# huangnengCSU/longcallR

Measured on AMD Instinct MI355X. Metric: candidate_sites_per_sec, higher is better.
Workload: dtype u8 in, u32 counts, f64 likelihoods, i64 fixed-point phase scores

## Files before the change

longcallr_amd/api.py:

```python
import ctypes as C

import numpy as np

from . import _abi, _lib
from ._lib import LcrError


def _view(ptr, dtype, n):
    if n == 0 or not ptr:
        return np.zeros(0, dtype=dtype)
    buf = (C.c_char * (np.dtype(dtype).itemsize * n)).from_address(ptr)
    return np.frombuffer(buf, dtype=dtype, count=n).copy()


def _view_nocopy(ptr, dtype, n):
    if n == 0 or not ptr:
        return np.zeros(0, dtype=dtype)
    buf = (C.c_char * (np.dtype(dtype).itemsize * n)).from_address(ptr)
    return np.frombuffer(buf, dtype=dtype, count=n)


_DEBUG_ENV = {"LCR_PHASE_PROF": "phase_prof", "LCR_GRID_MIN_ENTRIES": "grid_min_entries",
              "LCR_GRID_GENERIC": "grid_generic", "LCR_GRID_SPEC_LANES": "grid_spec_lanes", "LCR_GRID_SPEC_BATCH": "grid_spec_batch", "LCR_POST_HALF": "post_half", "LCR_ENUM_FORCE_BIG": "enum_force_big",
              "LCR_ENUM_FORCE_STREAM": "enum_force_stream", "LCR_ENUM_ELIDE": "enum_elide", "LCR_HIST_TILES": "hist_tiles", "LCR_TIE_ARITH": "tie_arith", "LCR_CHAIN_TIES": "chain_ties", "LCR_K3_HITS": "k3_hits", "LCR_FUSE_FILTER": "fuse_filter", "LCR_ASYNC_PHASE": "async_phase", "LCR_HOST_TRACE": "host_trace", "LCR_OWN_FILL": "own_fill", "LCR_REDO_LDS": "redo_lds", "LCR_SPEC_COMPACT": "spec_compact", "LCR_LEAN_PLANES": "lean_planes"}


class Engine:
    def __init__(self, device=0, params=None, timing=False):
        self.lib = _lib.load()
        h = C.c_void_p()
        rc = self.lib.lcr_ctx_create(device, C.byref(h))
        if rc != 0:
            raise LcrError("lcr_ctx_create(device=%d) failed with %d: no usable HIP device; "
                           "liblcr has no CPU fallback" % (device, rc))
        self.h = h
        self.device = device
        self.params = params if params is not None else _abi.make_params()
        self._sites = None
        self._keep = None
        self.last_truncated_columns = 0
        if timing:
            self.lib.lcr_enable_timing(self.h, 1)
            if timing is not True:
                self.debug_set("timing_mask", sum(1 << int(k) for k in timing))
        import os
        for env, key in _DEBUG_ENV.items():
            v = os.environ.get(env)
            if v is not None:
                self.debug_set(key, int(v) if v.lstrip("-").isdigit() else 1)
        if os.environ.get("LCR_LOCK_DIR"):
            self._chk(self.lib.lcr_ctx_set_lock_dir(self.h, os.fsencode(os.environ["LCR_LOCK_DIR"])), "lcr_ctx_set_lock_dir")

    def debug_set(self, key, value):
        self._chk(self.lib.lcr_debug_set(self.h, key.encode(), int(value)), "lcr_debug_set")
        return self

    def close(self):
        if getattr(self, "h", None):
            self.lib.lcr_ctx_destroy(self.h)
            self.h = None

    __del__ = close

    def _chk(self, rc, what):
        if rc != 0:
            raise LcrError("%s failed (%d): %s" % (what, rc, self.lib.lcr_last_error(self.h).decode()))

    def set_stream(self, hip_stream_ptr):
        self._chk(self.lib.lcr_ctx_set_stream(self.h, C.c_void_p(hip_stream_ptr)), "lcr_ctx_set_stream")

    def sync(self):
        self._chk(self.lib.lcr_ctx_sync(self.h), "lcr_ctx_sync")
        self._sites = None

    def set_async_phase(self, on=True):
        rc = self.lib.lcr_ctx_set_async_phase(self.h, 1 if on else 0)
        self.async_warning = self.lib.lcr_last_error(self.h).decode() if rc > 0 else None
        if rc < 0:
            self._chk(rc, "lcr_ctx_set_async_phase")
        return self

    def load_batch(self, batch):
        if isinstance(batch, _abi.ReadBatch):
            reads, regions = batch.c_reads(), batch.c_regions()
            self._keep = (batch, reads, regions)
        else:
            reads, regions, keep = batch
            self._keep = (keep, reads, regions)
        self._chk(self.lib.lcr_load_batch(self.h, C.byref(reads), C.byref(regions)), "lcr_load_batch")
        return self

    def load_batch_async(self, batch, slot):
        reads, regions = batch.c_reads(), batch.c_regions()
        if not hasattr(self, "_keep_slot"):
            self._keep_slot = {}
        self._chk(self.lib.lcr_load_batch_async(self.h, C.byref(reads), C.byref(regions), int(slot)), "lcr_load_batch_async")
        self._keep_slot[int(slot)] = (batch, reads, regions)
        return self

    def bind_batch(self, slot):
        self._chk(self.lib.lcr_bind_batch(self.h, int(slot)), "lcr_bind_batch")
        return self

    def discover_regions(self, ref_start, ref_end, contig_len, truncation=False, truncation_coverage=200000):
        if not 0 <= int(truncation_coverage) < 1 << 32:
            raise ValueError("truncation_coverage must be in [0, 2^32), got %r" % (truncation_coverage,))
        rs = np.ascontiguousarray(ref_start, dtype=np.int32)
        re_ = np.ascontiguousarray(ref_end, dtype=np.int32)
        o = _abi.LcrRegionList()
        nt = C.c_int64(0)
        self._chk(self.lib.lcr_discover_regions_truncated(self.h, _abi.LCR_MEM_HOST, int(rs.size), rs.ctypes.data, re_.ctypes.data,
                                                          int(contig_len), 1 if truncation else 0, int(truncation_coverage), C.byref(o),
                                                          C.byref(nt)), "lcr_discover_regions_truncated")
        self.last_truncated_columns = int(nt.value)
        return list(zip(_view(o.start0, np.int64, o.n_regions).tolist(), _view(o.len, np.int32, o.n_regions).tolist(),
                        _view(o.max_cov, np.uint32, o.n_regions).tolist()))

    def fill_data_into_freq_vec(self):
        self._chk(self.lib.lcr_pileup(self.h, C.byref(self.params)), "lcr_pileup")
        return self

    def get_candidate_snps(self):
        self._chk(self.lib.lcr_candidates(self.h, C.byref(self.params)), "lcr_candidates")
        return self

    def import_external_candidates(self, pos0, genotype, qual):
        if any(getattr(t, "is_cuda", False) for t in (pos0, genotype, qual)):
            import torch
            ts = (pos0, genotype, qual)
            want = (torch.int64, torch.uint8, torch.float32)
            if not all(getattr(t, "is_cuda", False) for t in ts):
                raise ValueError("device sites: pos0, genotype and qual must all be device tensors")
            for name, t, dt in zip(("pos0", "genotype", "qual"), ts, want):
                if t.dtype != dt:
                    raise ValueError("device sites: %s must be %s, got %s" % (name, dt, t.dtype))
                if t.device.index != self.device:
                    raise ValueError("device sites: %s is on %s, the engine on device %d" % (name, t.device, self.device))
                if t.dim() != 1 or not t.is_contiguous():
                    raise ValueError("device sites: %s must be a contiguous 1-d tensor" % name)
            if len({t.numel() for t in ts}) != 1:
                raise ValueError("pos0, genotype and qual must have the same length")
            self._release_sites()
            torch.cuda.current_stream(self.device).synchronize()
            self._chk(self.lib.lcr_import_candidates(self.h, C.byref(self.params), _abi.LCR_MEM_DEVICE, int(pos0.numel()),
                                                     *[C.c_void_p(t.data_ptr()) for t in ts]), "lcr_import_candidates")
            self._sites = ts
            return self
        p = np.ascontiguousarray(pos0, dtype=np.int64)
        g = np.ascontiguousarray(genotype, dtype=np.uint8)
        q = np.ascontiguousarray(qual, dtype=np.float32)
        if not (p.size == g.size == q.size):
            raise ValueError("pos0, genotype and qual must have the same length")
        self._release_sites()
        self._chk(self.lib.lcr_import_candidates(self.h, C.byref(self.params), _abi.LCR_MEM_HOST, int(p.size), p.ctypes.data, g.ctypes.data,
                                                 q.ctypes.data), "lcr_import_candidates")
        return self

    def _release_sites(self):
        if self._sites is not None:
            self.sync()

    def get_fragments(self):
        self._chk(self.lib.lcr_fragments(self.h, C.byref(self.params)), "lcr_fragments")
        self._sites = None
        return self

    def phase(self):
        self._chk(self.lib.lcr_phase(self.h, C.byref(self.params)), "lcr_phase")
        return self

    def junctions(self, min_count=10, min_junctions=2):
        p = _abi.LcrJunctionParams(int(min_count), int(min_junctions))
        self._chk(self.lib.lcr_junctions(self.h, C.byref(p)), "lcr_junctions")
        o = _abi.LcrJunctionList()
        self._chk(self.lib.lcr_get_junctions(self.h, C.byref(o)), "lcr_get_junctions")
        return _view(o.junc, _abi.JUNC_DTYPE, o.n_junctions), _view(o.junc_region_off, np.int32, o.n_regions + 1)

# ... 194 lines not shown
```

longcallr_amd/csrc/k4_enum.hip:

```cpp
#include <climits>
#include <type_traits>
#include "k4_dev.h"
#include "k4_grid.h"
#include "k4_kernels.h"

#ifndef ENUM_OCC
#define ENUM_OCC 3
#endif
namespace {

struct EnumTile { int32_t slot; uint32_t e0, ne; };
__device__ __forceinline__ EnumTile enum_tile_of(const PhaseDev& P, const EnumSpan* __restrict__ spans, int n_spans, uint32_t per, bool winner) {
  EnumTile t;
  const uint32_t bid = blockIdx.x;
  if (winner) { t.slot = spans[bid].slot; t.e0 = 0; t.ne = 1; return t; }
  const int lane = threadIdx.x & 63;
  int lo = 0, hi = n_spans;
  if (n_spans <= 4096) {
    const int step = (n_spans + 63) / 64;
    const int i1 = lane * step;
    const unsigned long long m1 = __ballot(i1 < n_spans && spans[min(i1, n_spans - 1)].tile0 <= bid);
    const int seg = __popcll(m1) - 1;
    lo = seg * step; hi = min(n_spans, lo + step);
    const int i2 = lo + lane;
    const unsigned long long m2 = __ballot(i2 < hi && spans[min(i2, n_spans - 1)].tile0 <= bid);
    lo = lo + __popcll(m2) - 1;
  } else {
    while (hi - lo > 1) { const int mid = (lo + hi) >> 1; if (spans[mid].tile0 <= bid) lo = mid; else hi = mid; }
  }
  t.slot = spans[lo].slot;
  const uint32_t n = 1u << P.reg[t.slot].S;
  t.e0 = (bid - spans[lo].tile0) * per;
  t.ne = min(per, n - t.e0);
  return t;
}

#if defined(ENUM_PROF) && ENUM_PROF == 2
#define ENUM_PROF_STEPS 1
#define ENUM_STEP(k) do { prof_steps[k] += (unsigned long long)E; } while (0)
#define ENUM_STEP_FLUSH(base) do { if (lane == 0) for (int k = 0; k < 4; k++) atomicAdd(&P.tie_ctr[(base) + k], prof_steps[k]); } while (0)
#else
#define ENUM_STEP(k) do { } while (0)
#define ENUM_STEP_FLUSH(base) do { } while (0)
#endif
#if defined(ENUM_PROF) && !defined(ENUM_PROF_STEPS)
#define ENUM_PROF_TIMES 1
#define ENUM_PT(i) do { if (threadIdx.x == 0) atomicMax(&P.tie_ctr[i], (unsigned long long)((long long)wall_clock64() - prof_t0)); } while (0)
#else
#define ENUM_PT(i) do { } while (0)
#endif
__global__ void __launch_bounds__(64 * ENUM_WAVES)
k4_enum_resolve(PhaseDev P, const EnumSpan* __restrict__ spans, const int64_t* __restrict__ job_base, const long long* __restrict__ job_obj,
                const int64_t* __restrict__ st_base, const unsigned long long* __restrict__ st_words) {
  extern __shared__ __attribute__((aligned(16))) uint8_t lds[];
  const long long prof_t0 = (long long)wall_clock64(); (void)prof_t0;
  const int slot = spans[blockIdx.x].slot;
  const RegionDev rd = P.reg[slot];
  const int tid = threadIdx.x, nt = blockDim.x, lane = tid & 63, wave = tid >> 6;
  const int R = rd.R, S = rd.S;
  const uint32_t E = (uint32_t)P.prow_ptr[rd.rp_off + R];
  const uint32_t n_jobs = 1u << S;
  const long long* const o = job_obj + job_base[slot];
  const unsigned long long* const st = st_words + st_base[slot];
  const uint32_t nk = (uint32_t)(R + 63) / 64, sw = enum_state_words((uint32_t)R);
  const ResolveLayout L = resolve_layout((uint32_t)R, E, (uint32_t)S);
  uint16_t* rp = (uint16_t*)(lds + L.rp);
  uint16_t* ent16 = (uint16_t*)(lds + L.ent16);
  double* lut = (double*)(lds + L.lut);
  double* pse = (double*)(lds + L.pse);
  unsigned long long* sg_ref = (unsigned long long*)(lds + L.sg_ref);
  unsigned long long* hetw = (unsigned long long*)(lds + L.hetw);
  unsigned long long* repmask = (unsigned long long*)(lds + L.repmask);
  uint32_t* rowsnps = (uint32_t*)(lds + L.rowsnps);
  __shared__ uint32_t s_adj[32], s_grp[32];
  uint32_t* t_e = (uint32_t*)(lds + L.res);
  double* t_sum = (double*)(lds + L.res + 8 * ENUM_TCAP);
  constexpr uint32_t EVCAP = 96;
  double* ev_t = (double*)(lds + L.res + 16 * ENUM_TCAP);
  uint16_t* ev_x = (uint16_t*)(lds + L.res + 16 * ENUM_TCAP + 8 * EVCAP);
  __shared__ uint32_t s_nev;
  __shared__ long long s_best[ENUM_WAVES];
  __shared__ uint32_t s_wcnt[ENUM_WAVES], s_dif[ENUM_WAVES], s_ntied;
  const uint32_t TLCAP = resolve_tlcap((uint32_t)S);
  uint16_t* tl = (uint16_t*)(lds + L.res + 16 * ENUM_TCAP + 96 * 10 + 16);
  __shared__ uint32_t s_win, s_wj[ENUM_WAVES], s_first;
  __shared__ double s_winsum, s_wsum[ENUM_WAVES];
  __shared__ int s_flat;
  auto ld_obj = [&](uint32_t e) { return o[e]; };
  auto ld_st = [&](uint32_t e, uint32_t w) { return st[(size_t)e * sw + w]; };
  if (tid < 64) lut[tid] = (tid & 31) < 31 ? (tid < 32 ? P.lut64->le[tid] : P.lut64->l1e[tid - 32]) : 0.0;
  { const int32_t* g_rp = P.prow_ptr + rd.rp_off; for (int r = tid; r <= R; r += nt) rp[r] = (uint16_t)g_rp[r]; }
  for (int e = tid; e < (int)E; e += nt) {
    const uint32_t v = P.pval[rd.e_off + e];
    ent16[e] = (uint16_t)(((uint32_t)P.pcol[rd.e_off + e] & 31u) | (v & 32u) | ((v & 31u) << 6));
  }
  __syncthreads();
  for (int r = tid; r < R; r += nt) if (rp[r + 1] > rp[r]) ent16[rp[r + 1] - 1] |= 0x800u;
  ENUM_PT(0);
  constexpr int OV = 4;
  long long ov[OV];
  long long best = LLONG_MIN;
#pragma unroll
  for (int k = 0; k < OV; k++) { const uint32_t e = (uint32_t)tid + (uint32_t)k * 256u; ov[k] = e < n_jobs ? ld_obj(e) : LLONG_MIN; }
#pragma unroll
  for (int k = 0; k < OV; k++) if (ov[k] > best) best = ov[k];
  for (uint32_t e = tid + OV * 256u; e < n_jobs; e += nt) { const long long v = ld_obj(e); if (v > best) best = v; }
  for (int d = 32; d >= 1; d >>= 1) { const long long ob = __shfl_xor(best, d, 64); if (ob > best) best = ob; }
  if (lane == 0) s_best[wave] = best;
  if (tid == 0) { s_ntied = 0; s_first = 0xffffffffu; }
  __syncthreads();
  for (int w = 0; w < ENUM_WAVES; w++) if (s_best[w] > best) best = s_best[w];
  for (uint32_t p0 = 0; p0 < n_jobs; p0 += 256u) {
    const uint32_t e = p0 + (uint32_t)tid;
    const long long v = p0 < OV * 256u ? ov[p0 >> 8] : (e < n_jobs ? ld_obj(e) : LLONG_MIN);
    const bool hit = e < n_jobs && v == best;
    const unsigned long long m = __ballot(hit);
    if (lane == 0) s_wcnt[wave] = (uint32_t)__popcll(m);
    __syncthreads();
    uint32_t off = s_ntied, tot = 0;
    for (int w = 0; w < ENUM_WAVES; w++) { if (w < wave) off += s_wcnt[w]; tot += s_wcnt[w]; }
    const uint32_t at = off + (uint32_t)__popcll(m & ((1ull << lane) - 1ull));
    if (hit && at < TLCAP) tl[at] = (uint16_t)e;
    if (hit && at == 0) s_first = e;
    __syncthreads();
    if (tid == 0) s_ntied += tot;
    __syncthreads();
  }
  const uint32_t n_tied_all = s_ntied, n_tied = min(n_tied_all, TLCAP);
  const uint32_t first = s_first;
  const unsigned long long sig0 = ld_st(first, nk + 2);
  uint32_t dif = 0;
  for (uint32_t j = tid; j < n_tied; j += nt) if (ld_st(tl[j], nk + 2) != sig0) dif = 1;
  dif = __ballot(dif != 0) ? 1u : 0u;
  if (lane == 0) s_dif[wave] = dif;
  if (n_tied_all > TLCAP || n_jobs > 65536u) {
    if (tid == 0) TIE_COUNT(P.tie_ctr, TIE_BEST_UNRES, 1ull);
    dif = 0;
    if (lane == 0) s_dif[wave] = 0;
  }
  if (tid == 0) { s_win = first; s_winsum = 0.0; s_flat = 1; }
  __syncthreads();
  for (int w = 0; w < ENUM_WAVES; w++) dif |= s_dif[w];
  ENUM_PT(1);
#ifdef ENUM_ABL_NOSUM
  dif = 0;
#endif
  if (dif && P.tie_arith < 1) { if (tid == 0) TIE_COUNT(P.tie_ctr, TIE_BEST_UNRES, 1ull); dif = 0; }
#ifdef ENUM_PROF_TIMES
  long long prof_t5 = 0;
  __shared__ uint32_t s_tloc[ENUM_WAVES], s_tfull[ENUM_WAVES];
  if (tid < ENUM_WAVES) { s_tloc[tid] = 0; s_tfull[tid] = 0; }
#endif
  if (dif) {
    if (tid == 0) TIE_COUNT(P.tie_ctr, TIE_BEST_F64, 1ull);
    const unsigned long long rm0 = ld_st(first, nk);
    const uint32_t r_dneg = (uint32_t)rm0, r_eta0 = (uint32_t)(rm0 >> 32), r_etap = (uint32_t)ld_st(first, nk + 1);
    { int empty = 0; for (int k = tid; k < R; k += nt) empty |= rp[k] == rp[k + 1] ? 1 : 0; if (empty) s_flat = 0; }
    for (uint32_t x = E + tid; x < ((E + 7u) & ~7u); x += nt) ent16[x] = 0;
    for (uint32_t k = tid; k < nk; k += nt) sg_ref[k] = ld_st(first, k);
    const bool rows_ok = true;
    if (tid < 32) s_adj[tid] = 0;
    __syncthreads();
    for (uint32_t k0 = wave * 64; k0 < (uint32_t)R; k0 += 64 * ENUM_WAVES) {
      const uint32_t k = k0 + lane;
      uint32_t ms = 0;
      if (k < (uint32_t)R) for (int x = rp[k]; x < rp[k + 1]; x++) ms |= 1u << (ent16[x] & 31u);
      if (k < (uint32_t)R) rowsnps[k] = ms;
      const uint32_t hs = ms & r_eta0;
      const unsigned long long m = __ballot(hs != 0);
      if (lane == 0) hetw[k0 >> 6] = m;
      const int rep = hs ? __ffs((int)hs) - 1 : -1;
      if (hs & (hs - 1)) for (uint32_t rest = hs; rest; rest &= rest - 1) atomicOr(&s_adj[__ffs((int)rest) - 1], hs);
      if (rows_ok) for (int i = 0; i < S; i++) { const unsigned long long mi = __ballot(rep == i); if (lane == 0) repmask[(uint32_t)i * nk + (k0 >> 6)] = mi; }
    }
    __syncthreads();
    if (wave == 0) {
      uint32_t g = lane < 32 && ((r_eta0 >> lane) & 1u) ? (1u << lane) | s_adj[lane & 31] : 0u;
      for (int round = 0; round < 5; round++)
        for (int j2 = 0; j2 < 32; j2++) { const uint32_t v = (uint32_t)__shfl((int)g, j2, 64); if ((g >> j2) & 1u) g |= v; }
      if (lane < 32) s_grp[lane] = g;
    }
    __syncthreads();
    ENUM_PT(2);
    const bool prefix_ok = true;
    auto full_sum = [&](const uint32_t e, const uint32_t dneg, const uint32_t eta0, const uint32_t etap) -> double {
      const uint32_t cm = (dneg & eta0) | (~etap & ~eta0);
      double acc = 0.0;
      if (s_flat) {
        unsigned long long wsg = ld_st(e, 0), wnext = 0;
        int k = 0;
        uint32_t sneg = 0u - ((uint32_t)wsg & 1u);
        const uint32_t E8 = (E + 7u) & ~7u;
        uint4 nxt = E8 ? *(const uint4*)ent16 : make_uint4(0, 0, 0, 0);
        for (uint32_t x = 0; x < E8; x += 8) {
          const uint4 raw = nxt;
          if (x + 8 < E8) nxt = *(const uint4*)(ent16 + x + 8);
          const uint32_t r[4] = {(uint32_t)__builtin_amdgcn_readfirstlane((int)raw.x), (uint32_t)__builtin_amdgcn_readfirstlane((int)raw.y),
                                 (uint32_t)__builtin_amdgcn_readfirstlane((int)raw.z), (uint32_t)__builtin_amdgcn_readfirstlane((int)raw.w)};
// ... 448 lines not shown
            if (enum_tie_row_flips(r_a + roff, (uint32_t)(win >> roff) & 1u, dneg, eta0, etap, rp, ent16, lut)) { fm |= 1ull << roff; nfl++; }
          }
          n_tie_flip += nfl;
          tflip = __ballot(nfl != 0) != 0;
          if (!any && tflip) n_step++;
        }
        if (fm) {
          atomicXor(&sgb[r_a >> 6], fm << wsh);
          if (wsh && (fm >> (64 - wsh))) atomicXor(&sgb[(r_a >> 6) + 1], fm >> (64 - wsh));
        }
        wave_lds_sync();
        if (!any) h_inc = false; else { h_inc = true; hg_inc = true; }
        need_delta = any || tflip || iters == 0;
        ENUM_STEP(0);
      } else {
        if (P.tie_arith < 2) n_tie_unres += last_tie; else n_tie_f64 += last_tie;
        h_inc = false; need_delta = false;
        ENUM_STEP(1);
      }
      if (!P.enum_elide || need_delta) {
        {
          constexpr int HB = 8;
          int cur = -1; int alo = 0, ahi = 0;
          auto del_batch = [&](const uint32_t* v8) {
            uint32_t sw[HB]; uint2 wq[HB];
#pragma unroll
            for (int x = 0; x < HB; x++) {
              const uint32_t row = v8[x] & 0xffffu;
              sw[x] = ((const uint32_t*)sgb)[row >> 5];
              wq[x] = wl2[(v8[x] >> 22) & 31u];
            }
#pragma unroll
            for (int x = 0; x < HB; x++) {
              const uint32_t v = v8[x];
              const int i = (v >> 16) & 31;
              const uint32_t hit = ((v >> 21) ^ (sw[x] >> (v & 31u)) ^ (dneg >> i)) & (v >> 31);
              if ((v >> 31) && i != cur) {
                if (alo | ahi) atomicAdd(&Macc[cur], (unsigned long long)(((long long)ahi << 23) + alo));
                cur = i; alo = 0; ahi = 0;
              }
              alo += __mul24((int)hit, (int)wq[x].x);
              ahi += __mul24((int)hit, (int)wq[x].y);
            }
          };
          for (int h = 0; h < n_del; h += HB) {
            uint32_t v8[HB];
#pragma unroll
            for (int x = 0; x < HB; x++) v8[x] = c0 + h + x < c1 ? csc[c0 + h + x] : 0;
            del_batch(v8);
          }
          if (alo | ahi) atomicAdd(&Macc[cur], (unsigned long long)(((long long)ahi << 23) + alo));
        }
        wave_lds_sync();
        bool changed = false, dtie = false;
        int d_new = (dneg >> lane) & 1u, h_new = ((eta0 >> lane) & 1u) ? 0 : (((etap >> lane) & 1u) ? 1 : -1);
        if (live) {
          const long long M = (long long)Macc[lane];
          Macc[lane] = 0;
          const long long N0 = cF + M + het, N1 = cF + cW - M + het;
          int ch = 0; long long nb = N0;
          if (N1 > nb) { ch = 1; nb = N1; }
          if (cRef > nb) { ch = 2; nb = cRef; }
          if (cVar > nb) { ch = 3; nb = cVar; }
          dtie = (int)(N0 == nb) + (int)(N1 == nb) + (int)(cRef == nb) + (int)(cVar == nb) > 1;
          const long long ncur = h_new == 0 ? N0 : (h_new == 1 ? cRef : cVar);
          changed = nb > ncur;
          if (ch == 1) d_new ^= 1;
          h_new = ch <= 1 ? 0 : (ch == 2 ? 1 : -1);
          obj_i = ch <= 1 ? nb - het : (ch == 2 ? cRef - P.lut.f_homref : cVar - P.lut.f_homvar);
        }
        const uint32_t dneg_n = (uint32_t)__ballot(lane < S && d_new);
        const uint32_t eta0_n = (uint32_t)__ballot(lane < S && h_new == 0);
        const uint32_t etap_n = (uint32_t)__ballot(lane < S && h_new == 1);
        const bool any2 = __ballot(changed) != 0;
        last_dtie = (uint32_t)__popcll(__ballot(dtie));
        n_dtie += last_dtie;
        need_sigma = dneg_n != dneg || eta0_n != eta0 || etap_n != etap;
        if (!any2 && need_sigma) n_step++;
        dneg = dneg_n; eta0 = eta0_n; etap = etap_n;
        wave_lds_sync();
        if (!any2) hg_inc = false; else { hg_inc = true; h_inc = true; }
        ENUM_STEP(2);
      } else {
        n_dtie += last_dtie;
        hg_inc = false; need_sigma = false;
        ENUM_STEP(3);
      }
      if (++iters > 20) break;
    }
    bool redone = false;
    if (redo && n_dtie + n_step != ev0 && P.tie_arith >= 3) {
      uint32_t at = 0;
      if (lane == 0) at = atomicAdd(&redo[0], 1u);
      at = (uint32_t)__builtin_amdgcn_readfirstlane((int)at);
      if (at < redo_cap) {
        if (lane == 0) { redo[4 + 2 * at] = (uint32_t)t.slot; redo[5 + 2 * at] = e; }
        const uint32_t dd = n_dtie - n_dtie0, ds = n_step - n_step0;
        n_dtie -= dd; n_step -= ds;
        redone = true;
      }
    }
    const long long total = wave_sum_ll_dpp(obj_i);
    const long long seen = __hip_atomic_load(&region_best[t.slot], __ATOMIC_RELAXED, __HIP_MEMORY_SCOPE_AGENT);
    const bool keep = __builtin_amdgcn_readfirstlane((int)(total >= seen)) != 0;
    if (total > seen && lane == 0 && !redone) (void)__hip_atomic_fetch_max(&region_best[t.slot], total, __ATOMIC_RELAXED, __HIP_MEMORY_SCOPE_AGENT);
    unsigned long long sig = 0;
    if (keep) {
      const unsigned long long w0 = sgb[r_a >> 6], w1 = sgb[(r_a >> 6) + 1];
      const unsigned long long win = (wsh ? (w0 >> wsh) | (w1 << (64 - wsh)) : w0);
      unsigned long long hs = 0;
      uint32_t word = 0; int nb = 0, widx = 0;
      auto sig_bit = [&](uint32_t v0, uint32_t v1) {
        const uint32_t m = v0 >> 24, i = m & 31u, roff = v1 >> 24, pbit = (m >> 5) & 1u;
        const uint32_t sneg = (uint32_t)(win >> roff) & 1u;
        const uint32_t match = ((eta0 >> i) & 1u) ? (pbit ^ sneg ^ ((dneg >> i) & 1u)) : (((etap >> i) & 1u) ? pbit : pbit ^ 1u);
        word |= (match & (m >> 7)) << nb;
        if (++nb == 32) { hs = mix64(hs ^ (word + (unsigned long long)(lane * 64 + widx + 1) * 0x9E3779B97F4A7C15ULL)); word = 0; nb = 0; widx++; }
      };
#ifndef ENUM_ABL_NOSIG
      for (int x0 = 0; x0 < n_sig; x0 += 4) {
        uint2 v[4];
#pragma unroll
        for (int u = 0; u < 4; u++) v[u] = s0 + x0 + u < s1 ? csr[s0 + x0 + u] : make_uint2(0, 0);
#pragma unroll
        for (int u = 0; u < 4; u++) sig_bit(v[u].x, v[u].y);
      }
#endif
      if (nb) hs = mix64(hs ^ (word + (unsigned long long)(lane * 64 + widx + 1) * 0x9E3779B97F4A7C15ULL));
      sig = (unsigned long long)wave_sum_ll((long long)hs);
    }
    unsigned long long* stp = st_reg + (size_t)e * stw;
    if (keep) for (int k = lane; k < nk; k += 64) stp[k] = sgb[k];
    if (lane == 0) {
      if (keep) { stp[nk] = (unsigned long long)dneg | ((unsigned long long)eta0 << 32); stp[nk + 1] = (unsigned long long)etap; stp[nk + 2] = sig; }
      job_obj[job_base[t.slot] + e] = total;
    }
    wave_lds_sync();
  };
  for (uint32_t kk = wave; kk < ne; kk += ENUM_WAVES) run_restart(t.e0 + kk);
  n_tie_f64 = (uint32_t)wave_sum_ll((long long)n_tie_f64); n_tie_flip = (uint32_t)wave_sum_ll((long long)n_tie_flip); n_tie_unres = (uint32_t)wave_sum_ll((long long)n_tie_unres);
  if (lane == 0) {
    if (n_tie_f64) TIE_COUNT(P.tie_ctr, TIE_SIGMA_F64, (unsigned long long)n_tie_f64);
    if (n_tie_flip) TIE_COUNT(P.tie_ctr, TIE_SIGMA_FLIPS, (unsigned long long)n_tie_flip);
    if (n_tie_unres) TIE_COUNT(P.tie_ctr, TIE_SIGMA_UNRES, (unsigned long long)n_tie_unres);
    if (n_dtie) TIE_COUNT(P.tie_ctr, TIE_DELTA_UNRES, (unsigned long long)n_dtie);
    if (n_step) TIE_COUNT(P.tie_ctr, TIE_STEP_UNRES, (unsigned long long)n_step);
  }
  ENUM_STEP_FLUSH(4);
}

__device__ __forceinline__ uint32_t enum_spread8(uint32_t x) { x = (x | (x << 4)) & 0x0F0Fu; x = (x | (x << 2)) & 0x3333u; x = (x | (x << 1)) & 0x5555u; return x; }
__device__ __forceinline__ int enum_mad24(int a, int b, int c) { int d; asm("v_mad_i32_i24 %0, %1, %2, %3" : "=v"(d) : "v"(a), "v"(b), "v"(c)); return d; }

#ifndef ENUM_BITS_OCC
#define ENUM_BITS_OCC 2
#endif
#ifndef ENUM_ITER_CAP
#define ENUM_ITER_CAP 20
#endif
__global__ void __launch_bounds__(64 * ENUM_WAVES, ENUM_BITS_OCC)
k4_enum_bits(PhaseDev P, const EnumSpan* __restrict__ spans, int32_t n_spans, uint32_t per, const int64_t* __restrict__ job_base,
             long long* __restrict__ job_obj, const int64_t* __restrict__ st_base, unsigned long long* __restrict__ st_words,
             long long* __restrict__ region_best, uint32_t* __restrict__ redo, uint32_t redo_cap) {
  extern __shared__ __attribute__((aligned(16))) uint8_t lds[];
  const EnumTile t = enum_tile_of(P, spans, n_spans, per, false);
  const RegionDev rd = P.reg[t.slot];
  const int R = rd.R, S = rd.S;
  const uint32_t E = (uint32_t)P.prow_ptr[rd.rp_off + R];
  const EnumLayout L = enum_layout(R, E, true, (uint32_t)S);
  const int Sp = (int)enum_bits_sp((uint32_t)S);
  uint2* wl2 = (uint2*)lds;
  double* lut = (double*)(lds + L.lut);
  uint2* csr = (uint2*)(lds + L.csr);
  uint32_t* csc = (uint32_t*)(lds + L.csc);
  uint16_t* rp = (uint16_t*)(lds + L.rp); uint16_t* first_row = (uint16_t*)(lds + L.first_row);
  uint16_t* ent16 = (uint16_t*)(lds + L.ent16);
  const int tid = threadIdx.x, nt = blockDim.x;
  const uint32_t c = enum_chunk(E);
  __shared__ long long s_cF[32], s_cW[32], s_cRef[32], s_cVar[32], s_het[32];
  __shared__ uint8_t s_live[32];
  if (tid < 32) {
    const long long w = tid < 31 ? P.lut.f1e[tid] - P.lut.fe[tid] : 0;
    wl2[tid] = make_uint2((uint32_t)w & 0x7fffffu, (uint32_t)(w >> 23) & 0xffffffu);
  }
  if (tid < 64) lut[tid] = (tid & 31) < 31 ? (tid < 32 ? P.lut64->le[tid] : P.lut64->l1e[tid - 32]) : 0.0;
  const int32_t* g_rp = P.prow_ptr + rd.rp_off;
  for (int r = tid; r <= R; r += nt) rp[r] = (uint16_t)g_rp[r];
  __shared__ int32_t cps[33];
  if (tid <= S && tid < 33) cps[tid] = P.ccol_ptr[rd.cp_off + tid];
  int eta_init = 0;
  if (tid < 32) {
    long long cF = 0, cW = 0, cRef = 0, cVar = 0, het = 0; bool live = false;
    if (tid < S) {
      const long long* sc = P.snp_const + 4ll * (rd.snp_off + tid);
      cF = sc[0]; cW = sc[1]; cRef = sc[2] + P.lut.f_homref; cVar = sc[3] + P.lut.f_homvar;
      const int n = P.ccol_ptr[rd.cp_off + tid + 1] - P.ccol_ptr[rd.cp_off + tid];
      het = P.lut.f_het0 - (long long)n * P.lut.f_log2;
      live = P.snp_fp[rd.snp_off + tid] != 0 && n > 0;
      eta_init = init_genotype(P.snp_vt[rd.snp_off + tid]);
    }
    s_cF[tid] = cF; s_cW[tid] = cW; s_cRef[tid] = cRef; s_cVar[tid] = cVar; s_het[tid] = het; s_live[tid] = live ? 1 : 0;
  }
  __shared__ uint32_t s_e0i, s_epi;
  if (tid < 64) {
    const uint32_t a = (uint32_t)__ballot(tid < S && tid < 32 && eta_init == 0), b = (uint32_t)__ballot(tid < S && tid < 32 && eta_init == 1);
    if (tid == 0) { s_e0i = a; s_epi = b; }
  }
  __syncthreads();
  for (int e = tid; e < (int)E; e += nt) {
    const uint32_t cv = P.cval[rd.e_off + e];
    int col = 0;
    for (int i = 0; i < S; i++) col += (int)((uint32_t)e >= (uint32_t)cps[i + 1]);
    csc[e] = (uint32_t)P.crow[rd.e_off + e] | ((uint32_t)col << 16) | ((cv & 32u) << 16) | ((cv & 31u) << 22) | 0x80000000u;
  }
  uint16_t* const perm = (uint16_t*)(lds + L.pos);
  uint16_t* const gof = perm + ((R + 3) & ~3);
  uint16_t* const kidx = (uint16_t*)(lds + L.state);
  __shared__ int s_cnt[3];
  __shared__ int s_lstart[32];
  __syncthreads();
  if (tid < 64) {
    const int ln = tid;
    const unsigned long long lt = (1ull << ln) - 1ull;
    int nS = 0;
    int tot[32];
#pragma unroll
    for (int Lk = 0; Lk < 32; Lk++) tot[Lk] = 0;
    for (int base = 0; base < R; base += 64) {
      const int r = base + ln;
      const int n = r < R ? min(31, (int)rp[r + 1] - (int)rp[r]) : 0;
      const unsigned long long bs = __ballot(n == 1);
      if (n == 1) kidx[r] = (uint16_t)(nS + __popcll(bs & lt));
      nS += __popcll(bs);
      if (__ballot(n >= 2)) {
#pragma unroll
        for (int Lk = 2; Lk < 32; Lk++) {
          if (Lk <= S) {
            const unsigned long long bm = __ballot(n == Lk);
            if (n == Lk) kidx[r] = (uint16_t)(tot[Lk] + __popcll(bm & lt));
            tot[Lk] += __popcll(bm);
          }
        }
      }
    }
    int mine = 0;
#pragma unroll
    for (int Lk = 2; Lk < 32; Lk++) if (ln == Lk) mine = tot[Lk];
    int longer = 0;
    for (int Lk = 31; Lk >= 2; Lk--) { const int tl = __shfl(mine, Lk, 64); if (ln == Lk) s_lstart[ln] = longer; longer += tl; }
    if (ln == 0) { s_cnt[0] = longer; s_cnt[2] = nS; }
  }
  __syncthreads();
  const int nM = s_cnt[0], nS = s_cnt[2], nG = (nM + 63) >> 6;
  for (int r = tid; r < R; r += nt) {
    const int n = min(31, (int)rp[r + 1] - (int)rp[r]);
    if (n >= 2) perm[s_lstart[n] + kidx[r]] = (uint16_t)r;
  }
  __syncthreads();
  if (tid < 64) {
    int carry = 0;
    for (int g0 = 0; g0 <= nG; g0 += 64) {
      const int g = g0 + tid;
      const int len = g < nG ? min(31, (int)rp[perm[64 * g] + 1] - (int)rp[perm[64 * g]]) : 0;
      const int inc = wave_incl_scan(len);
      if (g <= nG) gof[g] = (uint16_t)(carry + inc - len);
      carry += __builtin_amdgcn_readlane(inc, 63);
    }
  }
  __syncthreads();
  const int eM = 64 * (int)gof[nG];
  for (int x = tid; x < eM; x += nt) csr[x] = make_uint2(0u, 0u);
  __syncthreads();
  for (int r = tid; r < R; r += nt) {
    const int e0 = rp[r], e1 = rp[r + 1];
    if (e0 == e1) continue;
    int at, step;
    if (e1 - e0 >= 2) {
      const int k = s_lstart[min(31, e1 - e0)] + kidx[r];
      at = 64 * (int)gof[k >> 6] + (k & 63); step = 64;
    } else { perm[nM + kidx[r]] = (uint16_t)r; at = eM + kidx[r]; step = 1; }
    for (int e = e0; e < e1; e++) {
      const uint32_t v = P.pval[rd.e_off + e];
      const uint32_t meta = (uint32_t)P.pcol[rd.e_off + e] | (v & 32u) | (e + 1 == e1 ? 64u : 0u) | 128u;
      const uint2 w = wl2[v & 31u];
      csr[at + (e - e0) * step] = make_uint2(w.x | (meta << 24), w.y);
      ent16[e] = (uint16_t)((meta & 63u) | ((v & 31u) << 6) | (e + 1 == e1 ? 0x800u : 0u));
    }
  }
  __syncthreads();
  const int lane = tid & 63, wave = tid >> 6;
  uint8_t* const wst = lds + L.state + wave * L.stride;
  uint8_t* const sg8 = wst;
  unsigned long long* const Macc = (unsigned long long*)(wst + ((R + 15) & ~7u));
  uint2* const mt = (uint2*)(Macc + 8 * Sp);
  uint32_t* const ms = (uint32_t*)(mt + 32);
  uint32_t* const tq = ms + 24;
  uint32_t* const tq_n = tq + ENUM_TQ;
  __shared__ uint32_t s_tcnt[ENUM_WAVES][8];
  uint32_t* const tcnt = s_tcnt[wave];
  const int c0 = min((int)E, lane * (int)c), c1 = min((int)E, (lane + 1) * (int)c);
  const int n_del = (int)min(c, E);
  const uint32_t smask = S >= 32 ? 0xffffffffu : ((1u << S) - 1u);
  const uint32_t e0_init = s_e0i, ep_init = s_epi;
  const int nk = (R + 63) / 64;
  unsigned long long* const st_reg = st_words + st_base[t.slot];
  const uint32_t stw = enum_state_words((uint32_t)R);
  uint32_t n_tie_f64 = 0, n_tie_flip = 0, n_tie_unres = 0;
  uint32_t n_dtie = 0, n_step = 0;
#ifdef ENUM_PROF_STEPS
  unsigned long long prof_steps[4] = {0, 0, 0, 0};
#endif
  const int n_pass = (S + 7) >> 3;
  for (uint32_t g0 = 8u * wave; g0 < t.ne; g0 += 8u * ENUM_WAVES) {
    const uint32_t e_base = t.e0 + g0;
    const int nst = (int)min(8u, t.ne - g0);
    const uint32_t valid8 = (1u << nst) - 1u;
    if (lane < 8) { ms[lane] = (e_base + (uint32_t)lane) & smask; ms[8 + lane] = e0_init; ms[16 + lane] = ep_init; }
    {
      constexpr uint64_t G = 0x9E3779B97F4A7C15ULL;
      const uint64_t FA = (uint64_t)rd.F_all, RG = FA * G;
      const uint64_t a_0 = rd.seed + ((uint64_t)S + FA + (uint64_t)e_base * FA + 1ull) * G;
      const int32_t* const dord = P.draw_ord ? P.draw_ord + rd.sig_off : nullptr;
      uint64_t a_row = a_0 + (uint64_t)lane * G;
      for (int k = 0; k < nk; k++) {
        const int row = lane + 64 * k;
        uint32_t b = 0;
        uint64_t a = dord ? a_0 + (uint64_t)(row < R ? dord[row] : 0) * G : a_row;
#pragma unroll
        for (int s = 0; s < 8; s++) {
          uint64_t z = (a ^ (a >> 30)) * 0xBF58476D1CE4E5B9ULL;
          z ^= z >> 27;
          const uint32_t zl = (uint32_t)z, zh = (uint32_t)(z >> 32);
          const uint32_t top = __umulhi(zl, 0x133111EBu) + zl * 0x94D049BBu + zh * 0x133111EBu;
          b |= (uint32_t)((top >> 31) == 0) << s;
          a += RG;
        }
        if (row < R) sg8[row] = (uint8_t)b;
        a_row += 64ull * G;
      }
    }
    for (int k = lane; k < 8 * Sp; k += 64) Macc[k] = 0;
    if (lane == 0) tq_n[0] = 0;
    wave_lds_sync();
    uint32_t act = valid8, hinc = valid8, hginc = valid8;
    int iters = 0;
    uint32_t ev_d[8], ev_s[8];
#pragma unroll
    for (int s = 0; s < 8; s++) { ev_d[s] = 0; ev_s[s] = 0; }
    long long objl[4] = {0, 0, 0, 0};
    uint32_t need_sigma8 = 0xFFu, need_delta8 = 0xFFu;
    uint32_t ld_dt[8];
#pragma unroll
    for (int s = 0; s < 8; s++) ld_dt[s] = 0;
    while (act) {
      uint32_t any8 = 0, tflip8 = 0;
      if (!P.enum_elide || (need_sigma8 & act)) {
        if (lane < 32) {
          uint32_t dn = 0, h8 = 0, ep = 0;
#pragma unroll
          for (int s = 0; s < 8; s++) { dn |= ((ms[s] >> lane) & 1u) << s; h8 |= ((ms[8 + s] >> lane) & 1u) << s; ep |= ((ms[16 + s] >> lane) & 1u) << s; }
          mt[lane] = make_uint2(enum_spread8(h8) | (enum_spread8(dn) << 16), dn | (h8 << 8) | (ep << 16));
          if (lane < 8) tcnt[lane] = 0;
        }
        wave_lds_sync();
        {
          int alo[8], ahi[8];
#pragma unroll
          for (int s = 0; s < 8; s++) { alo[s] = 0; ahi[s] = 0; }
          for (int g = 0; g < nG; g++) {
            const int gb = __builtin_amdgcn_readfirstlane((int)gof[g]), Lg = __builtin_amdgcn_readfirstlane((int)gof[g + 1]) - gb;
            const int kq = 64 * g + lane;
            const int row = kq < nM ? (int)perm[kq] : 0;
            const uint32_t sgb = kq < nM ? (uint32_t)sg8[row] : 0u;
            const uint32_t sg16 = enum_spread8(sgb);
            const uint2* const pe = csr + 64 * gb + lane;
            uint32_t uacc = 0;
            for (int x0 = 0; x0 < Lg; x0 += 2) {
              const bool two = x0 + 1 < Lg;
              uint2 v[2]; uint32_t mmv[2];
              v[0] = pe[64 * x0]; v[1] = two ? pe[64 * (x0 + 1)] : make_uint2(0, 0);
              mmv[0] = mt[(v[0].x >> 24) & 31u].x; mmv[1] = mt[(v[1].x >> 24) & 31u].x;
#pragma unroll
              for (int u = 0; u < 2; u++) {
                if (u == 1 && !two) break;
                const uint32_t v0 = v[u].x, v1 = v[u].y;
                const uint32_t m = v0 >> 24;
                const uint32_t mm = mmv[u];
                const uint32_t use16 = (m & 128u) ? (mm & 0xFFFFu) : 0u;
                const uint32_t hit16 = (((m & 32u) ? 0x5555u : 0u) ^ sg16 ^ (mm >> 16)) & use16;
                const uint32_t code = use16 | ((hit16 ^ use16) << 1);
                uacc |= use16;
#pragma unroll
                for (int s = 0; s < 8; s++) {
                  const int sgn = __builtin_amdgcn_sbfe((int)code, 2 * s, 2);
                  alo[s] = enum_mad24(sgn, (int)v0, alo[s]); ahi[s] = enum_mad24(sgn, (int)v1, ahi[s]);
                }
              }
            }
            {
              uint32_t fl = 0, tie = 0;
#pragma unroll
              for (int s = 0; s < 8; s++) {
                const int top = ahi[s] + (alo[s] >> 23);
                fl |= (uint32_t)(top < 0) << s;
                tie |= (uint32_t)(top == 0 && (alo[s] & 0x7fffff) == 0 && ((uacc >> (2 * s)) & 1u)) << s;
                alo[s] = 0; ahi[s] = 0;
              }
              fl &= act; tie &= act;
              any8 |= fl;
              if (fl) sg8[row] = (uint8_t)(sgb ^ fl);
              if (tie) {
                for (uint32_t tt = tie; tt; tt &= tt - 1u) atomicAdd(&tcnt[__ffs((int)tt) - 1], 1u);
                if (P.tie_arith < 2) n_tie_unres += (uint32_t)__popc(tie);
                else {
                  n_tie_f64 += (uint32_t)__popc(tie);
                  if (rp[row + 1] - rp[row] > 2) {
                    const uint32_t at = atomicAdd(tq_n, 1u);
                    if (at < ENUM_TQ) tq[at] = (uint32_t)row | (tie << 16) | (sgb << 24);
                    else {
                      for (uint32_t tt = tie; tt; tt &= tt - 1u) {
                        const int s = __ffs((int)tt) - 1;
                        if (enum_tie_row_flips(row, (sgb >> s) & 1u, ms[s], ms[8 + s], ms[16 + s], rp, ent16, lut)) {
                          atomicXor((uint32_t*)(sg8 + (row & ~3)), 1u << (8 * (row & 3) + s));
                          n_tie_flip++; tflip8 |= 1u << s;
                        }
                      }
                    }
                  }
                }
              }
            }
          }
          for (int x0 = lane; x0 < nS; x0 += 4 * 64) {
            uint2 v[4]; int rw[4];
#pragma unroll
            for (int u = 0; u < 4; u++) { const int x = x0 + 64 * u; v[u] = x < nS ? csr[eM + x] : make_uint2(0, 0); rw[u] = x < nS ? (int)perm[nM + x] : 0; }
#pragma unroll
            for (int u = 0; u < 4; u++) {
              const uint32_t v0 = v[u].x, v1 = v[u].y;
              const uint32_t m = v0 >> 24, i = m & 31u;
              if (!(m & 128u)) continue;
              const int row = rw[u];
              const uint32_t sb = sg8[row], s16 = enum_spread8(sb);
              const uint32_t mm = mt[i].x;
              const uint32_t use16 = mm & 0xFFFFu;
              const uint32_t hit16 = (((m & 32u) ? 0x5555u : 0u) ^ s16 ^ (mm >> 16)) & use16;
              const bool wneg = ((v1 >> 23) & 1u) != 0;
              uint32_t f = wneg ? hit16 : (use16 & ~hit16);
              f &= 0x5555u; f = (f | (f >> 1)) & 0x3333u; f = (f | (f >> 2)) & 0x0F0Fu; f = (f | (f >> 4)) & 0xFFu;
              f &= act;
              any8 |= f;
              if (f) sg8[row] = (uint8_t)(sb ^ f);
            }
          }
        }
        wave_lds_sync();
// ... 68 lines not shown
              }
            }
          }
          if (cur >= 0) flush();
        }
        wave_lds_sync();
        {
          const int s = lane >> 3;
          const uint32_t od = ms[s], oe0 = ms[8 + s], oep = ms[16 + s];
          uint32_t nd = od, ne0 = oe0, nep = oep;
          for (int p = 0; p < n_pass; p++) {
            const int i = 8 * p + (lane & 7);
            const bool in = i < S;
            const bool live = in && s_live[i & 31] != 0;
            int d_new = (int)((od >> i) & 1u), h_new = ((oe0 >> i) & 1u) ? 0 : (((oep >> i) & 1u) ? 1 : -1);
            bool changed = false, dtie = false;
            if (live && ((act >> s) & 1u)) {
              const long long M = (long long)Macc[s * Sp + i];
              const long long cF = s_cF[i], cW = s_cW[i], cRef = s_cRef[i], cVar = s_cVar[i], het = s_het[i];
              const long long N0 = cF + M + het, N1 = cF + cW - M + het;
              int ch = 0; long long nb = N0;
              if (N1 > nb) { ch = 1; nb = N1; }
              if (cRef > nb) { ch = 2; nb = cRef; }
              if (cVar > nb) { ch = 3; nb = cVar; }
              dtie = (int)(N0 == nb) + (int)(N1 == nb) + (int)(cRef == nb) + (int)(cVar == nb) > 1;
              const long long ncur = h_new == 0 ? N0 : (h_new == 1 ? cRef : cVar);
              changed = nb > ncur;
              if (ch == 1) d_new ^= 1;
              h_new = ch <= 1 ? 0 : (ch == 2 ? 1 : -1);
              objl[p] = ch <= 1 ? nb - het : (ch == 2 ? cRef - P.lut.f_homref : cVar - P.lut.f_homvar);
            }
            if (in) Macc[s * Sp + i] = 0;
            const unsigned long long bd = __ballot(in && d_new), b0 = __ballot(in && h_new == 0), bp = __ballot(in && h_new == 1);
            const unsigned long long bc = __ballot(changed), bt = __ballot(dtie);
            const uint32_t sh = 8u * (uint32_t)s, keep = ~(0xFFu << (8 * p));
            nd = (nd & keep) | ((uint32_t)((bd >> sh) & 0xFFull) << (8 * p));
            ne0 = (ne0 & keep) | ((uint32_t)((b0 >> sh) & 0xFFull) << (8 * p));
            nep = (nep & keep) | ((uint32_t)((bp >> sh) & 0xFFull) << (8 * p));
#pragma unroll
            for (int q = 0; q < 8; q++) {
              if ((bc >> (8 * q)) & 0xFFull) any2 |= 1u << q;
              const uint32_t nt8 = (uint32_t)__popcll((bt >> (8 * q)) & 0xFFull);
              n_dtie += nt8; ev_d[q] += nt8; ld_dt[q] += nt8;
            }
          }
          nd &= smask; ne0 &= smask; nep &= smask;
          const bool frozen = !((act >> s) & 1u);
          if (frozen) { nd = od; ne0 = oe0; nep = oep; }
          const unsigned long long bm = __ballot(nd != od || ne0 != oe0 || nep != oep);
#pragma unroll
          for (int q = 0; q < 8; q++) if ((bm >> (8 * q)) & 0xFFull) chg8 |= 1u << q;
          wave_lds_sync();
          if ((lane & 7) == 0) { ms[s] = nd; ms[8 + s] = ne0; ms[16 + s] = nep; }
        }
        any2 &= act;
#pragma unroll
        for (int q = 0; q < 8; q++) if (((chg8 & ~any2 & act) >> q) & 1u) { n_step++; ev_s[q]++; }
        need_sigma8 = chg8;
        ENUM_STEP(2);
        wave_lds_sync();
      } else {
#pragma unroll
        for (int q = 0; q < 8; q++) if ((act >> q) & 1u) { n_dtie += ld_dt[q]; ev_d[q] += ld_dt[q]; }
        need_sigma8 = 0;
        ENUM_STEP(3);
      }
      hginc = (hginc & ~act) | (any2 & act); hinc |= any2 & act;
      iters++;
      act &= hinc | hginc;
      if (iters > ENUM_ITER_CAP) act = 0;
    }
    long long tot = objl[0] + objl[1] + objl[2] + objl[3];
    tot += __shfl_xor(tot, 1, 64); tot += __shfl_xor(tot, 2, 64); tot += __shfl_xor(tot, 4, 64);
    if (lane < 32) {
      uint32_t dn = 0, h8 = 0, ep = 0;
#pragma unroll
      for (int s = 0; s < 8; s++) { dn |= ((ms[s] >> lane) & 1u) << s; h8 |= ((ms[8 + s] >> lane) & 1u) << s; ep |= ((ms[16 + s] >> lane) & 1u) << s; }
      mt[lane] = make_uint2(0u, dn | (h8 << 8) | (ep << 16));
    }
    wave_lds_sync();
    unsigned long long hs[8];
    {
      uint32_t word[8];
#pragma unroll
      for (int s = 0; s < 8; s++) { hs[s] = 0; word[s] = 0; }
      int nb = 0, widx = 0;
      const int n_grp = (int)gof[nG], n_one = (nS + 63) / 64;
      int gq = 0;
      for (int x = 0; x < n_grp + n_one; x++) {
        const bool one = x >= n_grp;
        const int xs = lane + 64 * (x - n_grp);
        if (!one) while ((int)gof[gq + 1] <= x) gq++;
        const uint2 v = one ? (xs < nS ? csr[eM + xs] : make_uint2(0, 0)) : csr[64 * x + lane];
        const uint32_t m = v.x >> 24, i = m & 31u;
        const uint32_t y = mt[i].y, dn8 = y & 0xFFu, h8 = (y >> 8) & 0xFFu, ep8 = (y >> 16) & 0xFFu;
        const int srow = (m & 128u) ? (int)perm[one ? nM + xs : 64 * gq + lane] : 0;
        const uint32_t p8 = (m & 32u) ? 0xFFu : 0u, sn8 = sg8[srow];
        const uint32_t match = (m & 128u) ? ((h8 & (p8 ^ sn8 ^ dn8)) | (~h8 & ~(p8 ^ ep8))) & 0xFFu : 0u;
#pragma unroll
        for (int s = 0; s < 8; s++) word[s] |= ((match >> s) & 1u) << nb;
        if (++nb == 32) {
#pragma unroll
          for (int s = 0; s < 8; s++) { hs[s] = mix64(hs[s] ^ (word[s] + (unsigned long long)(lane * 64 + widx + 1) * 0x9E3779B97F4A7C15ULL)); word[s] = 0; }
          nb = 0; widx++;
        }
      }
      if (nb) {
#pragma unroll
        for (int s = 0; s < 8; s++) hs[s] = mix64(hs[s] ^ (word[s] + (unsigned long long)(lane * 64 + widx + 1) * 0x9E3779B97F4A7C15ULL));
      }
    }
#pragma unroll
    for (int s = 0; s < 8; s++) {
      if (s >= nst) break;
      const uint32_t e = e_base + (uint32_t)s;
      const long long total = ((long long)__builtin_amdgcn_readlane((int)(tot >> 32), 8 * s) << 32) | (unsigned int)__builtin_amdgcn_readlane((int)tot, 8 * s);
      bool redone = false;
      if (redo && ev_d[s] + ev_s[s] != 0 && P.tie_arith >= 3) {
        uint32_t at = 0;
        if (lane == 0) at = atomicAdd(&redo[0], 1u);
        at = (uint32_t)__builtin_amdgcn_readfirstlane((int)at);
        if (at < redo_cap) {
          if (lane == 0) { redo[4 + 2 * at] = (uint32_t)t.slot; redo[5 + 2 * at] = e; }
          n_dtie -= ev_d[s]; n_step -= ev_s[s];
          redone = true;
        }
      }
      const long long seen = __hip_atomic_load(&region_best[t.slot], __ATOMIC_RELAXED, __HIP_MEMORY_SCOPE_AGENT);
      const bool keep = __builtin_amdgcn_readfirstlane((int)(total >= seen)) != 0;
      if (total > seen && lane == 0 && !redone) (void)__hip_atomic_fetch_max(&region_best[t.slot], total, __ATOMIC_RELAXED, __HIP_MEMORY_SCOPE_AGENT);
      unsigned long long* stp = st_reg + (size_t)e * stw;
      if (keep) {
        const unsigned long long sig = (unsigned long long)wave_sum_ll((long long)hs[s]);
        for (int k = 0; k < nk; k++) {
          const int row = 64 * k + lane;
          const unsigned long long w = __ballot(row < R && ((sg8[min(row, max(R - 1, 0))] >> s) & 1u));
          if (lane == 0) stp[k] = w;
        }
        if (lane == 0) { stp[nk] = (unsigned long long)ms[s] | ((unsigned long long)ms[8 + s] << 32); stp[nk + 1] = (unsigned long long)ms[16 + s]; stp[nk + 2] = sig; }
      }
      if (lane == 0) job_obj[job_base[t.slot] + e] = total;
    }
    wave_lds_sync();
  }
  n_tie_f64 = (uint32_t)wave_sum_ll((long long)n_tie_f64); n_tie_flip = (uint32_t)wave_sum_ll((long long)n_tie_flip); n_tie_unres = (uint32_t)wave_sum_ll((long long)n_tie_unres);
  if (lane == 0) {
    if (n_tie_f64) TIE_COUNT(P.tie_ctr, TIE_SIGMA_F64, (unsigned long long)n_tie_f64);
    if (n_tie_flip) TIE_COUNT(P.tie_ctr, TIE_SIGMA_FLIPS, (unsigned long long)n_tie_flip);
    if (n_tie_unres) TIE_COUNT(P.tie_ctr, TIE_SIGMA_UNRES, (unsigned long long)n_tie_unres);
    if (n_dtie) TIE_COUNT(P.tie_ctr, TIE_DELTA_UNRES, (unsigned long long)n_dtie);
    if (n_step) TIE_COUNT(P.tie_ctr, TIE_STEP_UNRES, (unsigned long long)n_step);
  }
  ENUM_STEP_FLUSH(0);
}

__device__ __forceinline__ void enum_big_restart(const PhaseDev& P, const RegionDev& rd, int slot, uint32_t e, bool winner, int8_t* base, double* qrow,
                                                 long long* red, const long long* wl, unsigned long long* s_sig, const int64_t* __restrict__ job_base,
                                                 long long* __restrict__ job_obj, const int64_t* __restrict__ st_base, unsigned long long* __restrict__ st_words,
                                                 const MatView& mv, unsigned long long* macc = nullptr) {
  int8_t* sg = base; int8_t* dl = base + rd.R; int8_t* et = dl + rd.S;
  const int8_t* vt = P.snp_vt + rd.snp_off;
  const int lane = threadIdx.x & 63, wave = threadIdx.x >> 6;
  const uint32_t nk = (uint32_t)(rd.R + 63) / 64, sw = enum_state_words((uint32_t)rd.R);
  const bool keep = !winner && st_words && st_base[slot] >= 0;
  for (int i = threadIdx.x; i < rd.S; i += blockDim.x) { dl[i] = ((e >> i) & 1u) ? -1 : 1; et[i] = init_genotype(vt[i]); }
  const uint64_t ctr0 = (uint64_t)rd.S + (uint64_t)rd.F_all + (uint64_t)e * (uint64_t)rd.F_all;
  const int32_t* const dord = P.draw_ord ? P.draw_ord + rd.sig_off : nullptr;
  for (int row = threadIdx.x; row < rd.R; row += blockDim.x) sg[row] = u01(rd.seed, ctr0 + draw_row(dord, row)) < 0.5 ? -1 : 1;
  __syncthreads();
  const long long obj = cross_optimize(P, rd, mv, sg, dl, et, false, true, red, wl, macc, 32, nullptr, 0, nullptr, nullptr, nullptr, nullptr, qrow);
  if (winner) {
    for (int i = threadIdx.x; i < rd.S; i += blockDim.x) { P.st_delta[rd.snp_off + i] = dl[i]; P.st_eta[rd.snp_off + i] = et[i]; }
    for (int row = threadIdx.x; row < rd.R; row += blockDim.x) P.st_sigma[rd.sig_off + row] = sg[row];
    if (threadIdx.x == 0) P.st_obj[slot] = obj;
  } else {
    if (threadIdx.x == 0) job_obj[job_base[slot] + e] = obj;
    if (keep) {
      unsigned long long* dst = st_words + st_base[slot] + (size_t)e * sw;
      unsigned long long h = 0;
      for (uint32_t w0 = (uint32_t)wave; w0 < nk; w0 += LCR_BLOCK / 64) {
        const uint32_t row = 64u * w0 + (uint32_t)lane;
        const unsigned long long word = __ballot(row < (uint32_t)rd.R && sg[row] < 0);
        if (lane == 0) dst[w0] = word;
        h ^= mix64(word + 0x9E3779B97F4A7C15ull * (w0 + 1));
      }
      if (lane == 0) s_sig[wave] = h;
      __syncthreads();
      if (wave == 0) {
        const bool in = lane < rd.S;
        const unsigned long long dneg = __ballot(in && dl[in ? lane : 0] < 0), eta0 = __ballot(in && et[in ? lane : 0] == 0), etap = __ballot(in && et[in ? lane : 0] == 1);
        if (lane == 0) {
          const unsigned long long w0 = (dneg & 0xffffffffull) | (eta0 << 32), w1 = etap & 0xffffffffull;
          unsigned long long sig = mix64(w0 + 1) ^ mix64(w1 + 0x5851F42D4C957F2Dull);
          for (int w = 0; w < LCR_BLOCK / 64; w++) sig ^= s_sig[w];
          dst[nk] = w0; dst[nk + 1] = w1; dst[nk + 2] = sig;
        }
      }
    }
  }
  __syncthreads();
}
__global__ void __launch_bounds__(LCR_BLOCK)
k4_enum_big(PhaseDev P, const EnumSpan* __restrict__ spans, int32_t n_spans, uint32_t per, const int64_t* __restrict__ job_base,
            long long* __restrict__ job_obj, const uint32_t* __restrict__ win_e, const int64_t* __restrict__ st_base,
            unsigned long long* __restrict__ st_words, double* __restrict__ qrow, int64_t qrow_stride) {
  __shared__ long long red[LCR_BLOCK / 64];
  __shared__ long long wl[32];
  __shared__ unsigned long long s_sig[LCR_BLOCK / 64];
  const EnumTile t = enum_tile_of(P, spans, n_spans, per, win_e != nullptr);
  const RegionDev rd = P.reg[t.slot];
  load_w(P, wl);
  int8_t* base = P.scratch + (size_t)blockIdx.x * P.scratch_stride;
  double* qr = qrow ? qrow + (size_t)blockIdx.x * qrow_stride : nullptr;
  const uint32_t ne = win_e ? 1u : t.ne;
  for (uint32_t k = 0; k < ne; k++)
    enum_big_restart(P, rd, t.slot, win_e ? win_e[t.slot] : t.e0 + k, win_e != nullptr, base, qr, red, wl, s_sig, job_base, job_obj, st_base, st_words, global_view(P, rd));
}
__global__ void __launch_bounds__(LCR_BLOCK)
k4_enum_redo(PhaseDev P, const uint32_t* __restrict__ redo, uint32_t redo_cap, int8_t* __restrict__ scratch, int32_t scratch_stride, double* __restrict__ qrow,
             int64_t qrow_stride, const int64_t* __restrict__ job_base, long long* __restrict__ job_obj, const int64_t* __restrict__ st_base,
             unsigned long long* __restrict__ st_words, uint32_t lds_bytes) {
  __shared__ long long red[LCR_BLOCK / 64];
  __shared__ long long wl[32];
  __shared__ unsigned long long s_sig[LCR_BLOCK / 64];
  __shared__ unsigned long long macc[32];
  extern __shared__ __attribute__((aligned(16))) uint8_t redo_dyn[];
  const uint32_t n = min(redo[0], redo_cap);
  if (blockIdx.x >= n) return;
  load_w(P, wl);
  if (threadIdx.x < 32) macc[threadIdx.x] = 0;
  for (uint32_t i = blockIdx.x; i < n; i += gridDim.x) {
    const int slot = (int)redo[4 + 2 * i];
    const RegionDev rd = P.reg[slot];
    const uint32_t E = (uint32_t)P.prow_ptr[rd.rp_off + rd.R];
    const uint32_t st_b = ((uint32_t)(rd.R + 2 * rd.S) + 63u) & ~63u;
    __syncthreads();
    if (st_b + matview_bytes((uint32_t)rd.R, (uint32_t)rd.S, E) <= lds_bytes)
      enum_big_restart(P, rd, slot, redo[5 + 2 * i], false, reinterpret_cast<int8_t*>(redo_dyn), qrow + (size_t)blockIdx.x * qrow_stride,
                       red, wl, s_sig, job_base, job_obj, st_base, st_words, stage_view(P, rd, redo_dyn + st_b, E), macc);
    else
      enum_big_restart(P, rd, slot, redo[5 + 2 * i], false, scratch + (size_t)blockIdx.x * scratch_stride, qrow + (size_t)blockIdx.x * qrow_stride,
                       red, wl, s_sig, job_base, job_obj, st_base, st_words, global_view(P, rd));
  }
}

constexpr uint32_t TLB_CAP = 1024;
__global__ void __launch_bounds__(LCR_BLOCK)
k4_enum_resolve_big(PhaseDev P, const EnumSpan* __restrict__ spans, const int64_t* __restrict__ job_base, const long long* __restrict__ job_obj,
                    const int64_t* __restrict__ st_base, const unsigned long long* __restrict__ st_words, uint32_t* __restrict__ win_e,
                    double* __restrict__ terms, int64_t terms_stride) {
  __shared__ uint32_t tl[TLB_CAP];
  __shared__ unsigned long long sig[TLB_CAP];
  __shared__ double sum[TLB_CAP];
  __shared__ uint16_t rep[TLB_CAP];
  __shared__ double lut[64];
  __shared__ long long s_best[LCR_BLOCK / 64];
  __shared__ uint32_t s_wcnt[LCR_BLOCK / 64], s_ntied, s_first, s_dif;
  const int tid = threadIdx.x, lane = tid & 63, wave = tid >> 6;
  const int slot = spans[blockIdx.x].slot;
  const RegionDev rd = P.reg[slot];
  const int R = rd.R, S = rd.S;
  const uint32_t n_jobs = 1u << S, nk = (uint32_t)(R + 63) / 64, sw = enum_state_words((uint32_t)R);
  const long long* o = job_obj + job_base[slot];
  const bool have_st = st_words && st_base[slot] >= 0;
  const unsigned long long* st = st_words + (have_st ? st_base[slot] : 0);
  if (tid < 64) lut[tid] = (tid & 31) < 31 ? (tid < 32 ? P.lut64->le[tid] : P.lut64->l1e[tid - 32]) : 0.0;
  long long best = LLONG_MIN;
  for (uint32_t e = tid; e < n_jobs; e += LCR_BLOCK) { const long long v = o[e]; if (v > best) best = v; }
  for (int d = 32; d >= 1; d >>= 1) { const long long ob = __shfl_xor(best, d, 64); if (ob > best) best = ob; }
  if (lane == 0) s_best[wave] = best;
  if (tid == 0) { s_ntied = 0; s_first = 0xffffffffu; s_dif = 0; }
  __syncthreads();
  for (int w = 0; w < LCR_BLOCK / 64; w++) if (s_best[w] > best) best = s_best[w];
  for (uint32_t p0 = 0; p0 < n_jobs; p0 += LCR_BLOCK) {
    const uint32_t e = p0 + (uint32_t)tid;
    const bool hit = e < n_jobs && o[e] == best;
    const unsigned long long m = __ballot(hit);
    if (lane == 0) s_wcnt[wave] = (uint32_t)__popcll(m);
    __syncthreads();
    uint32_t off = s_ntied, tot = 0;
    for (int w = 0; w < LCR_BLOCK / 64; w++) { if (w < wave) off += s_wcnt[w]; tot += s_wcnt[w]; }
    const uint32_t at = off + (uint32_t)__popcll(m & ((1ull << lane) - 1ull));
    if (hit && at < TLB_CAP) tl[at] = e;
    if (hit && at == 0) s_first = e;
    __syncthreads();
    if (tid == 0) s_ntied += tot;
    __syncthreads();
  }
  const uint32_t n_all = s_ntied, n_tied = min(n_all, TLB_CAP), first = s_first;
  uint32_t win = first;
  if (n_all > 1) {
    if (!have_st || n_all > TLB_CAP || P.tie_arith < 1) { if (tid == 0) TIE_COUNT(P.tie_ctr, TIE_BEST_UNRES, 1ull); }
    else {
      for (uint32_t j = tid; j < n_tied; j += LCR_BLOCK) sig[j] = st[(size_t)tl[j] * sw + nk + 2];
      __syncthreads();
      for (uint32_t j = tid; j < n_tied; j += LCR_BLOCK) {
        uint32_t r = j;
        for (uint32_t i = 0; i < j; i++) if (sig[i] == sig[j]) { r = i; break; }
        rep[j] = (uint16_t)r;
        if (r != 0) s_dif = 1;
      }
      __syncthreads();
      if (s_dif) {
        if (tid == 0) TIE_COUNT(P.tie_ctr, TIE_BEST_F64, 1ull);
        const MatView mv = global_view(P, rd);
        const uint32_t E = (uint32_t)mv.rp[R];
        double* tb = terms + (size_t)blockIdx.x * terms_stride;
        for (uint32_t j = 0; j < n_tied; j++) {
          if (rep[j] != j) continue;
          const unsigned long long* cf = st + (size_t)tl[j] * sw;
          const unsigned long long rm0 = cf[nk];
          const uint32_t dneg = (uint32_t)rm0, eta0 = (uint32_t)(rm0 >> 32), etap = (uint32_t)cf[nk + 1];
          const uint32_t cm = (dneg & eta0) | (~etap & ~eta0);
          for (int row = tid; row < R; row += LCR_BLOCK) {
            const uint32_t sneg = 0u - (uint32_t)((cf[row >> 6] >> (row & 63)) & 1ull);
            for (int x = mv.rp[row]; x < mv.rp[row + 1]; x++) {
              const uint32_t i = (uint32_t)mv.pc[x], v = mv.pv[x];
              const uint32_t pbit = (v >> 5) & 1u, q = v & 31u;
              const uint32_t match = (pbit ^ (cm >> i) ^ ((sneg & eta0) >> i)) & 1u;
              tb[x] = lut[(match << 5) + q];
            }
          }
          __threadfence_block();
          __syncthreads();
          if (wave == 0) {
            double acc = 0.0;
            for (uint32_t b0 = 0; b0 < E; b0 += 64) {
              const double tv = b0 + (uint32_t)lane < E ? tb[b0 + lane] : 0.0;
              const int lo = (int)__double2loint(tv), hi = (int)__double2hiint(tv);
              const uint32_t n = min(64u, E - b0);
#pragma unroll 8
              for (uint32_t kk = 0; kk < 64; kk++)
                if (kk < n) acc += __hiloint2double(__builtin_amdgcn_readlane(hi, (int)kk), __builtin_amdgcn_readlane(lo, (int)kk));
            }
            if (lane == 0) sum[j] = acc;
          }
          __syncthreads();
        }
        if (tid == 0) {
          double bs = sum[0];
          for (uint32_t j = 1; j < n_tied; j++) { const double sj = sum[rep[j]]; if (sj > bs) { bs = sj; win = tl[j]; } }
          s_first = win;
        }
        __syncthreads();
        win = s_first;
      }
    }
  }
  if (tid == 0) win_e[slot] = win;
}
}

void launch_k4_enum_reg(unsigned n_blocks, size_t dyn_lds, hipStream_t s, const PhaseDev& P, const EnumSpan* spans, int32_t n_spans,
                        uint32_t per, const int64_t* job_base, long long* job_obj, const int64_t* st_base, unsigned long long* st_words,
                        long long* region_best, uint32_t* redo, uint32_t redo_cap) {
  hipLaunchKernelGGL(k4_enum_reg, dim3(n_blocks), dim3(64 * ENUM_WAVES), dyn_lds, s, P, spans, n_spans, per, job_base, job_obj, st_base, st_words, region_best, redo, redo_cap);
}
void launch_k4_enum_bits(unsigned n_blocks, size_t dyn_lds, hipStream_t s, const PhaseDev& P, const EnumSpan* spans, int32_t n_spans,
                         uint32_t per, const int64_t* job_base, long long* job_obj, const int64_t* st_base, unsigned long long* st_words,
                         long long* region_best, uint32_t* redo, uint32_t redo_cap) {
  hipLaunchKernelGGL(k4_enum_bits, dim3(n_blocks), dim3(64 * ENUM_WAVES), dyn_lds, s, P, spans, n_spans, per, job_base, job_obj, st_base, st_words, region_best, redo, redo_cap);
}
void launch_k4_enum_redo(unsigned n_blocks, hipStream_t s, const PhaseDev& P, const uint32_t* redo, uint32_t redo_cap, int8_t* scratch, int32_t scratch_stride,
                         double* qrow, int64_t qrow_stride, const int64_t* job_base, long long* job_obj, const int64_t* st_base, unsigned long long* st_words,
                         uint32_t lds_bytes) {
  lds_bytes = std::min<uint32_t>(lds_bytes, 128 * 1024);
  if (lds_bytes > 32 * 1024 && k4_set_dyn_lds_once(reinterpret_cast<const void*>(&k4_enum_redo), 128 * 1024, 6) != hipSuccess) { (void)hipGetLastError(); lds_bytes = 32 * 1024; }
  hipLaunchKernelGGL(k4_enum_redo, dim3(n_blocks), dim3(LCR_BLOCK), lds_bytes, s, P, redo, redo_cap, scratch, scratch_stride, qrow, qrow_stride, job_base, job_obj, st_base, st_words, lds_bytes);
}
void launch_k4_enum_resolve(unsigned n_regions, size_t dyn_lds, hipStream_t s, const PhaseDev& P, const EnumSpan* spans, const int64_t* job_base,
                            const long long* job_obj, const int64_t* st_base, const unsigned long long* st_words) {
  hipLaunchKernelGGL(k4_enum_resolve, dim3(n_regions), dim3(64 * ENUM_WAVES), dyn_lds, s, P, spans, job_base, job_obj, st_base, st_words);
}
void launch_k4_enum_big(unsigned n_blocks, hipStream_t s, const PhaseDev& P, const EnumSpan* spans, int32_t n_spans, uint32_t per,
                        const int64_t* job_base, long long* job_obj, const uint32_t* win_e, const int64_t* st_base, unsigned long long* st_words,
                        double* qrow, int64_t qrow_stride) {
  hipLaunchKernelGGL(k4_enum_big, dim3(n_blocks), dim3(LCR_BLOCK), 0, s, P, spans, n_spans, per, job_base, job_obj, win_e, st_base, st_words, qrow, qrow_stride);
}
void launch_k4_enum_resolve_big(int32_t n, hipStream_t s, const PhaseDev& P, const EnumSpan* spans, const int64_t* job_base, const long long* job_obj,
                                const int64_t* st_base, const unsigned long long* st_words, uint32_t* win_e, double* terms, int64_t terms_stride) {
  hipLaunchKernelGGL(k4_enum_resolve_big, dim3((unsigned)n), dim3(LCR_BLOCK), 0, s, P, spans, job_base, job_obj, st_base, st_words, win_e, terms, terms_stride);
}
```

longcallr_amd/csrc/k4_kernels.h:

```cpp
#pragma once
#include "k4_types.h"

struct EnumSpan { int32_t slot; uint32_t tile0; };
constexpr int ENUM_WAVES = 4;
constexpr uint32_t ENUM_LDS_MAX = 63 * 1024;

constexpr uint32_t ENUM_TQ = 126;
constexpr uint32_t ENUM_TCAP = 256;
#ifndef ENUM_BITS_PER_V
#define ENUM_BITS_PER_V 64
#endif
constexpr uint32_t ENUM_BITS_PER = ENUM_BITS_PER_V;
__host__ __device__ inline uint32_t enum_bits_sp(uint32_t S) { return (S + 7) & ~7u; }
__host__ __device__ inline uint32_t enum_bits_stride(uint32_t R, uint32_t S) { return ((R + 15) & ~7u) + 8 * 8 * enum_bits_sp(S) + 8 * 32 + 4 * 24 + 4 * (ENUM_TQ + 2); }
struct EnumLayout { uint32_t lut, csr, csc, rp, first_row, ent16, pos, state, stride, total; };
__host__ __device__ inline EnumLayout enum_layout(uint32_t R, uint32_t E, bool bits = false, uint32_t S = 32) {
  EnumLayout L;
  uint32_t o = 256;
  L.lut = o; o += 512;
  L.csr = o; o += 8 * (E + (bits ? 64 * (S < 31 ? S : 31) : 0));
  L.csc = o; o += 4 * E;
  L.rp = o; o += 2 * (R + 1);
  L.first_row = o; o += 2 * 65 + (bits ? 2 * 64 : 0);
  o = (o + 7) & ~7u;
  L.ent16 = o; o += 2 * ((E + 3) & ~3u);
  L.pos = o; if (bits) o += 2 * ((R + 3) & ~3u) + 2 * ((R + 4) & ~3u);
  o = (o + 15) & ~15u;
  L.state = o;
  L.stride = bits ? enum_bits_stride(R, S) : 8 * ((R + 63) / 64 + 1) + 8 * 32 + 4 * (ENUM_TQ + 2);
  o += ENUM_WAVES * L.stride;
  L.total = o;
  return L;
}
__host__ __device__ inline uint32_t enum_state_words(uint32_t R) { return (R + 63) / 64 + 3; }
__host__ __device__ inline uint32_t resolve_tlcap(uint32_t S) { return S >= 12 ? 4096u : (S < 6 ? 64u : (1u << S)); }
struct ResolveLayout { uint32_t lut, rp, ent16, pse, sg_ref, hetw, repmask, rowsnps, res, total; };
__host__ __device__ inline ResolveLayout resolve_layout(uint32_t R, uint32_t E, uint32_t S) {
  ResolveLayout L;
  const uint32_t nk = (R + 63) / 64;
  uint32_t o = 0;
  L.lut = o; o += 512;
  L.rp = o; o += 2 * (R + 2);
  o = (o + 15) & ~15u;
  L.ent16 = o; o += 2 * ((E + 7) & ~7u);
  o = (o + 15) & ~15u;
  L.pse = o; o += 8 * ((E + 8) & ~7u);
  L.sg_ref = o; o += 8 * (nk + 1);
  L.hetw = o; o += 8 * (nk + 1);
  L.repmask = o; o += 8 * nk * (S ? S : 1);
  L.rowsnps = o; o += 4 * (R + 1);
  o = (o + 7) & ~7u;
  L.res = o; o += ENUM_TCAP * 16 + 96 * 10 + 16 + 2 * resolve_tlcap(S);
  L.total = (o + 15) & ~15u;
  return L;
}
__host__ __device__ inline uint32_t enum_chunk(uint32_t E) { return E ? (E + 63) / 64 : 1; }

void launch_k4_enum_reg(unsigned n_blocks, size_t dyn_lds, hipStream_t s, const PhaseDev& P, const EnumSpan* spans, int32_t n_spans,
                        uint32_t per, const int64_t* job_base, long long* job_obj, const int64_t* st_base, unsigned long long* st_words,
                        long long* region_best, uint32_t* redo , uint32_t redo_cap);
void launch_k4_enum_bits(unsigned n_blocks, size_t dyn_lds, hipStream_t s, const PhaseDev& P, const EnumSpan* spans, int32_t n_spans,
                         uint32_t per, const int64_t* job_base, long long* job_obj, const int64_t* st_base, unsigned long long* st_words,
                         long long* region_best, uint32_t* redo, uint32_t redo_cap);
void launch_k4_enum_redo(unsigned n_blocks, hipStream_t s, const PhaseDev& P, const uint32_t* redo, uint32_t redo_cap, int8_t* scratch ,
                         int32_t scratch_stride, double* qrow , int64_t qrow_stride, const int64_t* job_base, long long* job_obj,
                         const int64_t* st_base, unsigned long long* st_words, uint32_t lds_bytes );
void launch_k4_enum_resolve(unsigned n_regions, size_t dyn_lds, hipStream_t s, const PhaseDev& P, const EnumSpan* spans, const int64_t* job_base,
                            const long long* job_obj, const int64_t* st_base, const unsigned long long* st_words);
void launch_k4_enum_big(unsigned n_blocks, hipStream_t s, const PhaseDev& P, const EnumSpan* spans, int32_t n_spans, uint32_t per,
                        const int64_t* job_base, long long* job_obj, const uint32_t* win_e ,
                        const int64_t* st_base , unsigned long long* st_words,
                        double* qrow , int64_t qrow_stride);
void launch_k4_enum_resolve_big(int32_t n, hipStream_t s, const PhaseDev& P, const EnumSpan* spans, const int64_t* job_base, const long long* job_obj,
                                const int64_t* st_base, const unsigned long long* st_words, uint32_t* win_e, double* terms ,
                                int64_t terms_stride);

constexpr int STAGE_THREADS = 256;
constexpr int STG_E = 8192, STG_R = 4096, STG_S = 512;
void launch_k4_stage(int32_t n_regions, hipStream_t s, const StageIn& in, const StageOut& out, const PhaseLutDev& lut);
constexpr int SAMPLE_THREADS = 1024;
void launch_k4_sample(int32_t n_slots, const int32_t* d_slots, const int32_t* d_row_region_off, const int64_t* d_start0, uint32_t depth, uint64_t seed,
                      uint8_t* d_sampled, hipStream_t s);

constexpr int CHAIN_THREADS = 1024;
constexpr int POST_MAX_ROWS = 8192, POST_MAX_ENTRIES = 8192, POST_MAX_SNPS = 512;
struct PostLayout { uint32_t sps, rpa, rpb, sflags, soflags, parent, qcnt, rptr, ecol, erow, cent, ccptr, eval, tag, asg, fp, lok, dirty, shap, sgt, svt, rcode, total; };
__host__ __device__ inline PostLayout post_layout(uint32_t nrow, uint32_t E, uint32_t S) {
  PostLayout L;
  uint32_t o = 64 * 8;
  L.sps = o; o += 8 * S;
  L.rpa = o; o += 8 * S; L.rpb = o; o += 8 * S;
  L.sflags = o; o += 4 * S; L.soflags = o; o += 4 * S; L.parent = o; o += 4 * S;
  L.qcnt = o; o += 4 * 16 * S;
  L.rptr = o; o += 2 * (nrow + 2);
  L.ecol = o; o += 2 * E; L.erow = o; o += 2 * E; L.cent = o; o += 2 * E;
  L.ccptr = o; o += 2 * (S + 2);
  L.eval = o; o += E;
  L.tag = o; o += nrow; L.asg = o; o += nrow; L.fp = o; o += nrow; L.lok = o; o += nrow;
  L.dirty = o; o += nrow;
  L.shap = o; o += S; L.sgt = o; o += S; L.svt = o; o += S; L.rcode = o; o += S;
  L.total = (o + 15) & ~15u;
  return L;
}
static_assert(CHAIN_THREADS / 2 == 2 * LCR_BLOCK, "k4_post has two instantiations");
hipError_t launch_k4_post(int threads, unsigned n_blocks, size_t dyn_lds, hipStream_t s, const PostIn& in, const int32_t* slots, int32_t n_slots,
                          const PostLut& lut);
```

longcallr_amd/csrc/k4_phase.hip:

```cpp
#include <algorithm>
#include <chrono>
#include <cstdio>
#include <cstdlib>
#include <cmath>
#include <cstring>
#include <climits>
#include <map>
#include <mutex>
#include <fcntl.h>
#include <sys/file.h>
#include <unistd.h>
#include <sys/stat.h>
#include <cerrno>

#include "k4_dev.h"
#include "k4_grid.h"
#include "k4_post.h"
#include "k4_kernels.h"

namespace {


struct HostLut {
  double le[31], l1e[31];
  double p_homref, p_homvar, log_theta, log2;
  PhaseLutDev dev;
  HostLut() {
    for (int q = 0; q <= 30; q++) {
      const int qq = q == 0 ? 1 : q;
      const double eps = std::pow(10.0, -(double)qq / 10.0);
      le[q] = std::log10(eps); l1e[q] = std::log10(1.0 - eps);
      dev.fe[q] = std::llround(le[q] * FX_SCALE); dev.f1e[q] = std::llround(l1e[q] * FX_SCALE);
    }
    p_homref = std::log10(1.0 - 1.5 * 0.001); p_homvar = std::log10(0.5 * 0.001);
    log_theta = std::log10(0.001); log2 = std::log10(2.0);
    dev.f_homref = std::llround(p_homref * FX_SCALE); dev.f_homvar = std::llround(p_homvar * FX_SCALE);
    dev.f_het0 = std::llround(log_theta * FX_SCALE); dev.f_log2 = std::llround(log2 * FX_SCALE);
  }
};
const HostLut& hlut() { static HostLut l; return l; }

}

struct GridLock {
  int fd = -1;
  bool held = false;
  std::mutex* dev_mu = nullptr;
  hipStream_t q[3] = {nullptr, nullptr, nullptr};
  int n_q = 0;
  static std::mutex& device_mutex(const std::string& bus) {
    static std::mutex table_mu;
    static std::map<std::string, std::mutex*> table;
    std::lock_guard<std::mutex> g(table_mu);
    auto it = table.find(bus);
    if (it == table.end()) it = table.emplace(bus, new std::mutex()).first;
    return *it->second;
  }
  std::string acquire(const std::string& lock_dir, hipStream_t a, hipStream_t b, hipStream_t c) {
    if (held) return "";
    q[0] = a; q[1] = b; q[2] = c; n_q = 3;
    int dev = 0;
    char bus[64] = "gpu";
    if (hipGetDevice(&dev) == hipSuccess) (void)hipDeviceGetPCIBusId(bus, sizeof(bus), dev);
    for (char* ch = bus; *ch; ch++) if (*ch == ':' || *ch == '/') *ch = '_';
    std::string dir = lock_dir;
    bool shared = dir.empty();
    auto trusted = [&](const std::string& d) {
      struct stat st;
      if (lstat(d.c_str(), &st) != 0 || !S_ISDIR(st.st_mode)) return false;
      if (st.st_uid != getuid() && st.st_uid != 0) return false;
      return !(st.st_mode & 0022) || (st.st_mode & S_ISVTX) || st.st_uid == getuid();
    };
    if (shared) {
      dir = "/tmp/liblcr-locks";
      if (mkdir(dir.c_str(), 01777) == 0) (void)chmod(dir.c_str(), 01777);
      if (!trusted(dir)) return "the machine-wide lock directory " + dir + " exists but is not root's or this user's (or is writable by others without the sticky bit): "
                                "remove it, have an administrator create it 1777, or name a directory all processes that share this GPU see with lcr_ctx_set_lock_dir";
    }
    if (!shared && mkdir(dir.c_str(), 0700) != 0 && errno != EEXIST) return "cannot create lock directory " + dir + ": " + strerror(errno);
    if (!trusted(dir)) return "lock directory " + dir + " is not a directory of this user or of root (sticky if others may write): lcr_ctx_set_lock_dir names another one";
    const std::string path = dir + "/grid_" + bus + ".lock";
    dev_mu = &device_mutex(bus);
    dev_mu->lock();
    auto fail = [&](const std::string& e) { if (fd >= 0) { close(fd); fd = -1; } dev_mu->unlock(); dev_mu = nullptr; return e; };
    const auto t_start = std::chrono::steady_clock::now();
    for (;;) {
      fd = open(path.c_str(), O_CREAT | O_RDWR | O_NOFOLLOW | O_CLOEXEC, shared ? 0666 : 0600);
      if (fd < 0) return fail("cannot open " + path + ": " + strerror(errno));
      if (shared) { struct stat fs; if (fstat(fd, &fs) == 0 && fs.st_uid == getuid()) (void)fchmod(fd, 0666); }
      int rc;
      while ((rc = flock(fd, LOCK_EX | LOCK_NB)) != 0 && (errno == EWOULDBLOCK || errno == EINTR)) {
        if (std::chrono::duration<double>(std::chrono::steady_clock::now() - t_start).count() > 600.0)
          return fail("the device lock " + path + " has been held by another process for 10 minutes");
        usleep(200);
      }
      if (rc != 0) return fail("flock(" + path + "): " + strerror(errno));
      struct stat fa, fb;
      if (fstat(fd, &fa) == 0 && stat(path.c_str(), &fb) == 0 && fa.st_ino == fb.st_ino && fa.st_dev == fb.st_dev) break;
      (void)flock(fd, LOCK_UN); close(fd); fd = -1;
    }
    held = true;
    return "";
  }
  ~GridLock() {
    if (!held) return;
    for (int i = 0; i < n_q; i++) (void)hipStreamSynchronize(q[i]);
    if (fd >= 0) { (void)flock(fd, LOCK_UN); close(fd); }
    if (dev_mu) dev_mu->unlock();
  }
};

int PhaseHost::ld_blocks(const PhaseInputs& in, int region, std::vector<int32_t>* off, std::vector<int32_t>* snps, hipStream_t s, std::string* err) {
  off->assign(1, 0); snps->clear();
  for (const ChainDesc& d : chain_desc) {
    if (d.slot != region) continue;
    const int c0 = in.cand_region_off[region];
    int32_t info[2] = {0, 0};
    auto chk = [&](hipError_t e) { if (e != hipSuccess && err) *err = hipGetErrorString(e); return e == hipSuccess; };
    if (!chk(hipMemcpyAsync(info, chain_dev.blk_info + 2 * region, 8, hipMemcpyDeviceToHost, s)) || !chk(hipStreamSynchronize(s))) return LCR_E_DEVICE;
    const int nb = info[0];
    if (nb == 0) return LCR_OK;
    std::vector<int32_t> ptr(nb + 1);
    if (!chk(hipMemcpyAsync(ptr.data(), chain_dev.blk_ptr + c0 + region, (size_t)(nb + 1) * 4, hipMemcpyDeviceToHost, s)) || !chk(hipStreamSynchronize(s))) return LCR_E_DEVICE;
    std::vector<int32_t> nodes(ptr[nb]);
    if (!chk(hipMemcpyAsync(nodes.data(), chain_dev.blk_nodes + c0, (size_t)ptr[nb] * 4, hipMemcpyDeviceToHost, s)) || !chk(hipStreamSynchronize(s))) return LCR_E_DEVICE;
    for (int b = nb - 1; b >= 0; b--) {
      snps->insert(snps->end(), nodes.begin() + ptr[b], nodes.begin() + ptr[b + 1]);
      off->push_back((int32_t)snps->size());
    }
    return LCR_OK;
  }
  return LCR_OK;
}

#define PCHK_TO(err_, expr) do { hipError_t e_ = (expr); if (e_ != hipSuccess) { if (err_) *(err_) = std::string(#expr) + ": " + hipGetErrorString(e_); return LCR_E_DEVICE; } } while (0)
#define PCHK(expr) PCHK_TO(c.err, expr)
#define RCHK(expr) do { const int rc_ = (expr); if (rc_) return rc_; } while (0)
int PhaseHost::settle(std::string* err) {
  if (!pending) return LCR_OK;
  pending = false;
  PCHK_TO(err, hipStreamSynchronize(side));
  PCHK_TO(err, hipMemcpyAsync(h_census.p, d_tie.p, TIE_NCTR * 8, hipMemcpyDeviceToHost, q_first));
  PCHK_TO(err, hipStreamSynchronize(q_first));
  PCHK_TO(err, hipGetLastError());
  memcpy(tie_census, h_census.p, TIE_NCTR * 8);
  uint8_t* const h_r = h_res.as<uint8_t>();
  const long long* const h_obj = (const long long*)(h_cand_obj.as<uint8_t>() + pend.hc_obj);
  std::vector<lcr_candidate>& cand = *pend.cand;
  for (int g = 0; g < pend.ng; g++) {
    const int c0 = pend.cand_off[g], S = pend.cand_off[g + 1] - c0;
    if (S == 0) continue;
    memcpy(cand.data() + c0, h_cand_obj.as<lcr_candidate>() + c0, (size_t)S * sizeof(lcr_candidate));
    objective[g] = (double)h_obj[g] / FX_SCALE;
  }
  r_haplotag = (int8_t*)(h_r + pend.res_tag); r_assignment = h_r + pend.res_asg; r_phase_set = (uint32_t*)(h_r + pend.res_ps);
  return LCR_OK;
}

constexpr uint32_t REDO_CAP = 8192, REDO_GRID = 512;
constexpr uint32_t ENUM_STREAM_PER_WAVE = 2;

struct PhaseCall {
  const PhaseInputs& in; const lcr_params& prm; std::string* const err;
  const hipStream_t sq;
  const int ng, nrow, ncand; const int64_t nnz; const size_t nnz1, nc1, nr1; const bool prof;
  std::chrono::steady_clock::time_point t_last = std::chrono::steady_clock::now();
  bool async_mode = false; hipStream_t stream = nullptr;
  size_t st_sig = 0, st_del = 0, st_eta = 0, st_obj = 0, st_bytes = 0;
  size_t res_ps = 0, res_tag = 0, res_asg = 0, res_bytes = 0, hc_obj = 0;
  PhaseDev P{}, Pc{};
  PostIn pin{}, pinc{}; PostLut plut;
  StageIn si{}; StageOut so{};
  int64_t grid_min = 0; StageStat* stat = nullptr;
  std::vector<int32_t> enum_slots, chain_slots, gpost_slots, gstage_slots;
  std::vector<uint8_t> grid_post;
  uint32_t post_lds = 0;
  size_t gp_S = 1, gp_rows = 1, gp_E = 1;
  GridLock grid_lock;
  PhaseCall(const PhaseInputs& in_, const lcr_params& prm_, hipStream_t user_stream, std::string* err_, bool prof_)
      : in(in_), prm(prm_), err(err_), sq(user_stream), ng(in_.n_regions), nrow(in_.n_rows), ncand(in_.cand_region_off[in_.n_regions]),
        nnz(in_.nnz), nnz1((size_t)std::max<int64_t>(nnz, 1)), nc1((size_t)std::max(ncand, 1)), nr1((size_t)std::max(nrow, 1)), prof(prof_) {}
  void lap(const char* what) { if (!prof) return; auto t = std::chrono::steady_clock::now(); fprintf(stderr, "[phase] %-28s %8.3f ms\n", what, std::chrono::duration<double, std::milli>(t - t_last).count()); t_last = t; }
  int lock_grid(const PhaseHost& h) {
    const std::string e = grid_lock.acquire(h.lock_dir, stream, h.side, h.aux);
    if (!e.empty() && err) *err = "device lock of the persistent launches: " + e;
    return e.empty() ? LCR_OK : LCR_E_DEVICE;
  }
};

int PhaseHost::run(const PhaseInputs& in, const lcr_params& prm, hipStream_t user_stream, std::string* err) {
  RCHK(settle(err));
  HT("phase");
  PhaseCall c(in, prm, user_stream, err, dbg.prof != 0);
  objective.assign(c.ng, 0.0);
  RCHK(open_queues(c));
  RCHK(size_buffers(c));
  RCHK(sample(c));
  RCHK(stage(c));
  RCHK(classify(c));
  RCHK(wait_sizes(c));
  RCHK(launch_enum(c));
  HT("ph:enum_q");
  RCHK(launch_chain(c));
  c.lap("enum launch");
  RCHK(launch_gpost(c));
  c.lap("chain launch");
  if (!mark_pending(c)) return LCR_OK;
  PCHK_TO(err, hipStreamSynchronize(side));
  c.lap("chain kernels");
  RCHK(settle(err));
  c.lap("enumeration kernels");
  if (c.prof) RCHK(report_prof(c));
  c.lap("results");
  return LCR_OK;
}

int PhaseHost::open_queues(PhaseCall& c) {
  c.async_mode = dbg.async_phase != 0;
  if (c.async_mode && !main_q) PCHK(hipStreamCreateWithFlags(&main_q, hipStreamNonBlocking));
  if (!ev_user) { PCHK(hipEventCreateWithFlags(&ev_user, hipEventDisableTiming)); PCHK(hipEventCreateWithFlags(&ev_gate[0], hipEventDisableTiming)); PCHK(hipEventCreateWithFlags(&ev_gate[1], hipEventDisableTiming)); }
  gate_set[0] = gate_set[1] = false;
  c.stream = c.async_mode ? main_q : c.sq;
  q_first = c.stream;
  if (!side) {
    PCHK(hipStreamCreateWithFlags(&side, hipStreamNonBlocking));
    PCHK(hipEventCreateWithFlags(&ev_in, hipEventDisableTiming));
    PCHK(hipEventCreateWithFlags(&ev_csr, hipEventDisableTiming));
    PCHK(hipStreamCreateWithFlags(&aux, hipStreamNonBlocking));
    PCHK(hipEventCreateWithFlags(&ev_fork, hipEventDisableTiming));
    PCHK(hipEventCreateWithFlags(&ev_join, hipEventDisableTiming));
  }
  return LCR_OK;
}

int PhaseHost::size_buffers(PhaseCall& c) {
  const int ng = c.ng; const size_t nnz1 = c.nnz1, nc1 = c.nc1, nr1 = c.nr1;
  const HostLut& L = hlut();
  PCHK(d_reg.reserve((size_t)std::max(ng, 1) * sizeof(RegionDev)));
  PCHK(d_prow_ptr.reserve((nr1 + ng + 1) * 4)); PCHK(d_pcol.reserve(nnz1 * 4)); PCHK(d_pval.reserve(nnz1));
  PCHK(d_ccol_ptr.reserve((nc1 + ng + 1) * 4)); PCHK(d_crow.reserve(nnz1 * 4)); PCHK(d_cval.reserve(nnz1));
  PCHK(d_snp.reserve(nc1 * 3 + 16)); PCHK(d_snp_const.reserve(nc1 * 4 * sizeof(long long))); PCHK(d_cur.reserve(nc1 * 4));
  PCHK(d_prow_src.reserve(nr1 * 4));
  c.st_sig = 0; c.st_del = (nr1 + 15) & ~(size_t)15; c.st_eta = c.st_del + ((nc1 + 15) & ~(size_t)15);
  c.st_obj = c.st_eta + ((nc1 + 15) & ~(size_t)15); c.st_bytes = c.st_obj + (size_t)std::max(ng, 1) * 8;
  PCHK(d_st_enum.reserve(c.st_bytes + 16)); PCHK(d_st_chain.reserve(c.st_bytes + 16));
  PCHK(h_stat.reserve((size_t)std::max(ng, 1) * sizeof(StageStat)));
  c.res_ps = 0; c.res_tag = nr1 * 4; c.res_asg = nr1 * 5; c.res_bytes = nr1 * 6;
  c.hc_obj = (nc1 * sizeof(lcr_candidate) + 15) & ~(size_t)15;
  PCHK(h_res.reserve(c.res_bytes)); PCHK(h_cand_obj.reserve(c.hc_obj + (size_t)std::max(ng, 1) * 8));
  PCHK(d_read_rec.reserve(nr1 * 12));
  uint8_t* d_res = nullptr; uint8_t* d_hc = nullptr;
  PCHK(hipHostGetDevicePointer((void**)&d_res, h_res.p, 0));
  PCHK(hipHostGetDevicePointer((void**)&d_hc, h_cand_obj.p, 0));

  PhaseDev& P = c.P;
  P.reg = d_reg.as<RegionDev>();
  P.prow_ptr = d_prow_ptr.as<int32_t>(); P.pcol = d_pcol.as<int32_t>(); P.pval = d_pval.as<uint8_t>();
  P.ccol_ptr = d_ccol_ptr.as<int32_t>(); P.crow = d_crow.as<int32_t>(); P.cval = d_cval.as<uint8_t>();
  P.snp_const = d_snp_const.as<long long>();
  P.snp_fp = d_snp.as<uint8_t>(); P.snp_vt = d_snp.as<int8_t>() + nc1; P.snp_cons = d_snp.as<uint8_t>() + 2 * nc1;
  P.st_sigma = d_st_enum.as<int8_t>() + c.st_sig; P.st_delta = d_st_enum.as<int8_t>() + c.st_del; P.st_eta = d_st_enum.as<int8_t>() + c.st_eta;
  P.st_obj = (long long*)(d_st_enum.as<int8_t>() + c.st_obj);
  P.lut = L.dev;
  PostLut& plut = c.plut;
  for (int q = 0; q < 31; q++) { plut.le[q] = L.le[q]; plut.l1e[q] = L.l1e[q]; }
  plut.p_homref = L.p_homref; plut.p_homvar = L.p_homvar; plut.log_theta = L.log_theta; plut.log2 = L.log2;
  PCHK(d_lut64.reserve(sizeof(PostLut))); PCHK(d_tie.reserve(TIE_NCTR * 8)); PCHK(h_census.reserve(TIE_NCTR * 8));
  if (!lut64_ready) { PCHK(hipMemcpyAsync(d_lut64.p, &plut, sizeof(PostLut), hipMemcpyHostToDevice, c.sq)); PCHK(hipStreamSynchronize(c.sq)); lut64_ready = true; }
  PCHK(d_en_rbest.reserve((size_t)std::max(ng, 1) * 8 + 64));
  if (dbg.tie_arith >= 3) PCHK(d_en_redo.reserve(2 * (16 + 8 * (size_t)REDO_CAP) + 64));
  { void* const fp[4] = {d_tie.p, d_st_enum.p, d_en_rbest.p, d_en_redo.p};
    const int fv[4] = {0, 0, 0x80, 0};
    const size_t fs[4] = {TIE_NCTR * 8, ng ? c.st_bytes : 0, (size_t)ng * 8, dbg.tie_arith >= 3 ? 2 * (16 + 8 * (size_t)REDO_CAP) : 0};
    PCHK(lcr_fill_multi_async(4, fp, fv, fs, c.sq)); }
  P.lut64 = d_lut64.as<PostLut>(); P.tie_ctr = d_tie.as<unsigned long long>(); P.tie_arith = dbg.tie_arith; P.enum_elide = dbg.enum_elide;

  c.Pc = P;
  c.Pc.st_sigma = d_st_chain.as<int8_t>() + c.st_sig; c.Pc.st_delta = d_st_chain.as<int8_t>() + c.st_del; c.Pc.st_eta = d_st_chain.as<int8_t>() + c.st_eta;
  c.Pc.st_obj = (long long*)(d_st_chain.as<int8_t>() + c.st_obj);
  const PhaseInputs& in = c.in; const lcr_params& prm = c.prm;
  c.pin = PostIn{in.d_row_ptr, in.d_col, in.d_val, in.d_row_links, const_cast<lcr_candidate*>(in.d_cand), in.d_cand_off,
                 in.d_row_region_off, in.d_start0, P.st_sigma, P.st_delta, P.st_eta, (int8_t*)(d_res + c.res_tag), d_res + c.res_asg,
                 (uint32_t*)(d_res + c.res_ps), d_read_rec.as<uint32_t>(), P.st_obj, (long long*)(d_hc + c.hc_obj), (lcr_candidate*)d_hc,
                 prm.min_linkers, prm.max_enum_snps, prm.seed, prm.read_assign_cutoff, prm.min_phase_score, nullptr, P.reg, d_prow_src.as<int32_t>()};
  c.pinc = c.pin;
  c.pinc.st_sigma = c.Pc.st_sigma; c.pinc.st_delta = c.Pc.st_delta; c.pinc.st_eta = c.Pc.st_eta; c.pinc.st_obj = c.Pc.st_obj;
  return LCR_OK;
}

int PhaseHost::sample(PhaseCall& c) {
  const PhaseInputs& in = c.in;
  ds_applied.assign((size_t)std::max(c.ng, 1), 0); ds_any = false;
  ds_ng = (int32_t)c.ng; ds_nrow = (int32_t)c.nrow;
  if (!in.ds_rows && in.ds_depth == 0) return LCR_OK;
  PCHK(h_smp_slots.reserve((size_t)std::max(c.ng, 1) * 4));
  int32_t* const slots = h_smp_slots.as<int32_t>();
  int n = 0;
  for (int g = 0; g < c.ng; g++) {
    const int r0 = in.row_region_off[g], F = in.row_region_off[g + 1] - r0;
    bool app = false;
    if (in.ds_rows) app = F > 0 && memchr(in.ds_rows + r0, 0, (size_t)F) != nullptr;
    else app = F > 0 && (uint32_t)F >= in.ds_depth;
    if (app) { ds_applied[g] = 1; slots[n++] = g; }
  }
  if (!n) return LCR_OK;
  ds_any = true;
  PCHK(d_sampled.reserve(c.nr1)); PCHK(h_sampled.reserve(c.nr1)); PCHK(d_prow_ord.reserve(c.nr1 * 4));
  if (in.ds_rows) {
    memcpy(h_sampled.p, in.ds_rows, (size_t)c.nrow);
    PCHK(hipMemcpyAsync(d_sampled.p, h_sampled.p, (size_t)c.nrow, hipMemcpyHostToDevice, c.sq));
  } else {
    int32_t* d_slots = nullptr;
    PCHK(hipHostGetDevicePointer((void**)&d_slots, slots, 0));
    PCHK(lcr_fill_async(d_sampled.p, 1, (size_t)c.nrow, c.sq));
    launch_k4_sample(n, d_slots, in.d_row_region_off, in.d_start0, in.ds_depth, in.ds_seed, d_sampled.as<uint8_t>(), c.sq);
    PCHK(hipGetLastError());
    PCHK(hipMemcpyAsync(h_sampled.p, d_sampled.p, (size_t)c.nrow, hipMemcpyDeviceToHost, c.sq));
  }
  c.P.draw_ord = c.Pc.draw_ord = d_prow_ord.as<int32_t>();
  c.pin.sampled = c.pinc.sampled = d_sampled.as<uint8_t>();
  return LCR_OK;
}

int PhaseHost::stage(PhaseCall& c) {
  const PhaseInputs& in = c.in;
  c.grid_min = dbg.grid_min >= 0 ? dbg.grid_min : (1 << 17);
  c.stat = h_stat.as<StageStat>();
  c.si = StageIn{in.d_row_ptr, in.d_col, in.d_val, in.d_row_links, in.d_cand, in.d_cand_off, in.d_row_region_off, in.d_start0,
                 c.prm.min_linkers, c.prm.max_enum_snps, c.prm.seed, std::max<int64_t>(c.grid_min, 1), ds_any ? d_sampled.as<uint8_t>() : nullptr};
  if (!c.ng) return LCR_OK;
  StageStat* d_stat = nullptr;
  PCHK(hipHostGetDevicePointer((void**)&d_stat, c.stat, 0));
  c.so = StageOut{d_reg.as<RegionDev>(), d_stat, d_prow_ptr.as<int32_t>(), d_pcol.as<int32_t>(), d_pval.as<uint8_t>(),
                  d_ccol_ptr.as<int32_t>(), d_crow.as<int32_t>(), d_cval.as<uint8_t>(), d_snp.as<uint8_t>(), d_snp.as<int8_t>() + c.nc1,
                  d_snp.as<uint8_t>() + 2 * c.nc1, d_snp_const.as<long long>(), d_cur.as<int32_t>(), d_prow_src.as<int32_t>(),
                  ds_any ? d_prow_ord.as<int32_t>() : nullptr};
  launch_k4_stage((int32_t)c.ng, c.sq, c.si, c.so, hlut().dev);
  PCHK(hipGetLastError());
  HT("  ph:stage_q");
  return LCR_OK;
}

int PhaseHost::classify(PhaseCall& c) {
  const PhaseInputs& in = c.in;
  for (int g = 0; g < c.ng; g++) {
    const int S = in.snps(g);
    if (S == 0) continue;
    if ((uint32_t)S <= c.prm.max_enum_snps) c.enum_slots.push_back(g); else c.chain_slots.push_back(g);
  }
  c.grid_post.assign(c.ng, 0);
  for (int g = 0; g < c.ng; g++) {
    const int S = in.snps(g);
    if (S == 0) continue;
    const int nr_g = in.row_region_off[g + 1] - in.row_region_off[g];
    const int64_t E_all = in.region_e_off[g + 1] - in.region_e_off[g];
    if (E_all > INT_MAX - 64) { if (c.err) *c.err = "a region's fragment matrix has more than 2^31 entries"; return LCR_E_ARG; }
    if (E_all >= std::max<int64_t>(c.grid_min, 1)) c.gstage_slots.push_back(g);
    bool fits = !(nr_g > POST_MAX_ROWS || E_all > POST_MAX_ENTRIES || S > POST_MAX_SNPS);
    uint32_t need = 0;
    if (fits) { need = post_layout(nr_g, (uint32_t)E_all, S).total; if (need > 64 * 1024) fits = false; }
    if (!fits || (c.grid_min == 0 && (uint32_t)S > c.prm.max_enum_snps)) {
      c.grid_post[g] = 1; c.gpost_slots.push_back(g);
      c.gp_S = std::max(c.gp_S, (size_t)S); c.gp_rows = std::max(c.gp_rows, (size_t)nr_g); c.gp_E = std::max(c.gp_E, (size_t)E_all);
    } else c.post_lds = std::max(c.post_lds, need);
  }
  return LCR_OK;
}

int PhaseHost::wait_sizes(PhaseCall& c) {
  hipStream_t const sq = c.sq;
  PCHK(hipEventRecord(ev_in, sq));
  PCHK(hipStreamWaitEvent(side, ev_in, 0));
  if (c.ng) {
    if (!c.gstage_slots.empty()) {
      RCHK(c.lock_grid(*this));
      PCHK(d_grid_ctl.reserve((4 + 16) * sizeof(GridCtl))); PCHK(d_grid_tot.reserve((size_t)(3 * std::max(1, k4_grid_blocks()) + 1) * 4 + 64));
      for (int g : c.gstage_slots) PCHK(k4_stage_launch_grid(c.si, c.so, hlut().dev, g, d_grid_ctl.as<GridCtl>(), d_grid_tot.as<int32_t>(), side));
      PCHK(hipEventRecord(ev_join, side));
      PCHK(hipStreamWaitEvent(sq, ev_join, 0));
    }
    PCHK(hipEventRecord(ev_csr, sq));
  }
  if (c.async_mode) { PCHK(hipEventRecord(ev_user, sq)); PCHK(hipStreamWaitEvent(c.stream, ev_user, 0)); }
  HT("ph:presync");
  if (c.ng) PCHK(hipStreamSynchronize(sq));
  HT("ph:synced");
  c.lap("stage + sizes");
  const size_t clk_bytes = ((size_t)(c.ng + 1) * 16 + 2 * 1024) * 8;
  if (c.prof) { PCHK(d_prof_clk.reserve(clk_bytes)); PCHK(hipMemsetAsync(d_prof_clk.p, 0, clk_bytes, c.stream)); c.pin.dbg_clk = c.pinc.dbg_clk = d_prof_clk.as<long long>(); }
  return LCR_OK;
}

int PhaseHost::launch_enum(PhaseCall& c) {
  if (c.enum_slots.empty()) return LCR_OK;
  const PhaseInputs& in = c.in; const int ng = c.ng; const StageStat* const stat = c.stat;
  std::vector<int32_t>& enum_slots = c.enum_slots; PhaseDev& P = c.P; hipStream_t const stream = c.stream;
  {
    std::vector<uint64_t>& key = enum_keys;
    key.resize(enum_slots.size());
    for (size_t k = 0; k < enum_slots.size(); k++) key[k] = ((uint64_t)(0xffffffffu - (uint32_t)stat[enum_slots[k]].E) << 32) | (uint32_t)enum_slots[k];
    std::sort(key.begin(), key.end());
    for (size_t k = 0; k < enum_slots.size(); k++) enum_slots[k] = (int32_t)(uint32_t)key[k];
  }
  HT("en:sorted");
  int32_t max_state = 0;
  for (int g : enum_slots) max_state = std::max(max_state, stat[g].R + 2 * in.snps(g));
  const int32_t stride = (max_state + 63) & ~63;
  P.scratch_stride = stride;
  const bool force_big = dbg.enum_force_big != 0;
  const bool force_stream = dbg.enum_force_stream != 0;
  enum { CL_STREAM, CL_BITS, CL_BIG, NCLS };
  std::vector<EnumSpan> spans[NCLS];
  spans[CL_STREAM].reserve(enum_slots.size()); spans[CL_BITS].reserve(enum_slots.size());
  size_t n_t[NCLS] = {0, 0, 0};
  const uint32_t per_of[NCLS] = {ENUM_STREAM_PER_WAVE * ENUM_WAVES, ENUM_BITS_PER, 1u};
  std::vector<int64_t>& job_base = enum_job_base; std::vector<int64_t>& st_base = enum_st_base;
  job_base.assign(ng, 0); st_base.assign(ng, 0);
  int64_t nj = 0, st_words = 0, big_words = 0, big_emax = 0;
  uint32_t lds_need[NCLS] = {0, 0, 0}, res_lds[NCLS] = {0, 0, 0};
  std::vector<int32_t> post_slots, post_slots_b, post_slots_c;
  post_slots.reserve(enum_slots.size());
  for (int g : enum_slots) {
    const int S = in.snps(g);
    const StageStat& st = stat[g];
    const EnumLayout EL_stream = enum_layout(st.R, st.E), EL_bits = enum_layout(st.R, st.E, true, (uint32_t)std::min(S, 32));
    const bool use_bits = !force_stream && S <= 31 && EL_bits.total <= ENUM_LDS_MAX;
    const EnumLayout EL = use_bits ? EL_bits : EL_stream;
    const uint32_t RL = resolve_layout((uint32_t)st.R, (uint32_t)st.E, (uint32_t)S).total;
    int cls = CL_BIG;
    if (!force_big && st.R < 65536 && st.E < 65536 && S <= 31 && EL.total <= ENUM_LDS_MAX && RL <= ENUM_LDS_MAX && st.max_rows <= 64)
      cls = use_bits ? CL_BITS : CL_STREAM;
    if (cls != CL_BIG && (int64_t)((uint64_t)1 << std::min(S, 62)) * enum_state_words((uint32_t)st.R) > ((int64_t)1 << 27)) cls = CL_BIG;
    if (cls != CL_BIG) { lds_need[cls] = std::max(lds_need[cls], EL.total); res_lds[cls] = std::max(res_lds[cls], RL); }
    job_base[g] = nj;
    const uint64_t n = 1ull << S;
    st_base[g] = -1;
    if (cls != CL_BIG) { st_base[g] = st_words; st_words += (int64_t)n * enum_state_words((uint32_t)st.R); }
    else if ((int64_t)n * enum_state_words((uint32_t)st.R) <= ((int64_t)1 << 26) - big_words) {
      st_base[g] = st_words; st_words += (int64_t)n * enum_state_words((uint32_t)st.R); big_words += (int64_t)n * enum_state_words((uint32_t)st.R);
      big_emax = std::max<int64_t>(big_emax, st.E);
    }
    if (n_t[cls] + (n + per_of[cls] - 1) / per_of[cls] > 0x7fffffffull) { if (c.err) *c.err = "too many enumeration restarts for one launch"; return LCR_E_ARG; }
    spans[cls].push_back({g, (uint32_t)n_t[cls]});
    n_t[cls] += (size_t)((n + per_of[cls] - 1) / per_of[cls]);
    nj += (int64_t)n;
    if (!c.grid_post[g]) (cls == CL_BITS ? post_slots_b : (cls == CL_BIG ? post_slots_c : post_slots)).push_back(g);
    if (c.prof && cls == CL_BIG) fprintf(stderr, "[phase]   global-memory enumeration region %d: R %d E %d S %d max_rows %d max_n %d, LDS image %u B\n", g, st.R, st.E, S, st.max_rows, st.max_n, EL.total);
  }
  if (c.prof) fprintf(stderr, "[phase]   enumeration classes: bit states %zu regions / %zu tiles, streaming %zu / %zu, global %zu / %zu\n",
                      spans[CL_BITS].size(), n_t[CL_BITS], spans[CL_STREAM].size(), n_t[CL_STREAM], spans[CL_BIG].size(), n_t[CL_BIG]);
  size_t n_w[NCLS], s_off[NCLS], n_spans = 0;
  for (int k = 0; k < NCLS; k++) { n_w[k] = spans[k].size(); s_off[k] = n_spans; n_spans += n_w[k]; }
  const size_t ns = enum_slots.size(), nps_a = post_slots.size(), nps_b = post_slots_b.size(), nps_c = post_slots_c.size(), nps = nps_a + nps_b + nps_c;
  const size_t off_jb_al = (n_spans * sizeof(EnumSpan) + 7) & ~(size_t)7;
  const size_t off_sb = off_jb_al + (size_t)ng * 8;
  const size_t up_bytes = off_sb + (size_t)ng * 8 + (ns + nps) * 4;
  HT("en:classes");
  PCHK(d_en_st.reserve((size_t)std::max<int64_t>(st_words, 1) * 8));
  PCHK(d_en_job.reserve(up_bytes + 64));
  PCHK(d_en_obj.reserve((size_t)nj * 8 + (size_t)ng * 8 + (size_t)ng * 8 + 64));
  PCHK(h_en_up.reserve(up_bytes + 64));
  uint8_t* const up = h_en_up.as<uint8_t>();
  for (int k = 0; k < NCLS; k++) memcpy(up + s_off[k] * sizeof(EnumSpan), spans[k].data(), n_w[k] * sizeof(EnumSpan));
  memcpy(up + off_jb_al, job_base.data(), (size_t)ng * 8);
  memcpy(up + off_sb, st_base.data(), (size_t)ng * 8);
  memcpy(up + off_sb + (size_t)ng * 8, enum_slots.data(), ns * 4);
  memcpy(up + off_sb + (size_t)ng * 8 + ns * 4, post_slots.data(), nps_a * 4);
  memcpy(up + off_sb + (size_t)ng * 8 + (ns + nps_a) * 4, post_slots_b.data(), nps_b * 4);
  memcpy(up + off_sb + (size_t)ng * 8 + (ns + nps_a + nps_b) * 4, post_slots_c.data(), nps_c * 4);
  PCHK(hipMemcpyAsync(d_en_job.p, up, up_bytes, hipMemcpyHostToDevice, stream));
  HT("en:up_q");
  const EnumSpan* d_sp = d_en_job.as<EnumSpan>();
  const int64_t* d_jb = (const int64_t*)(d_en_job.as<uint8_t>() + off_jb_al);
  const int64_t* d_sb = (const int64_t*)(d_en_job.as<uint8_t>() + off_sb);
  const int32_t* d_sl = (const int32_t*)(d_en_job.as<uint8_t>() + off_sb + (size_t)ng * 8);
  const int32_t* d_psl = d_sl + ns;
  long long* d_obj = d_en_obj.as<long long>();
  uint32_t* d_win = (uint32_t*)(d_obj + nj);
  const size_t n_big_blocks = std::max(n_t[CL_BIG], n_w[CL_BIG]);
  const bool full_ties = dbg.tie_arith >= 3;
  int32_t max_rows_any = 1;
  for (int g : enum_slots) max_rows_any = std::max(max_rows_any, stat[g].R);
  const int64_t qstride = ((int64_t)2 * max_rows_any + 15) & ~(int64_t)15;
  const size_t n_scr_blocks = n_big_blocks + 2 * (size_t)REDO_GRID;
  PCHK(d_en_scr.reserve((size_t)stride * n_scr_blocks + 64));
  P.scratch = d_en_scr.as<int8_t>();
  if (full_ties) PCHK(d_en_qrow.reserve((size_t)qstride * n_scr_blocks * 8 + 64));
  uint32_t* const redo_a = full_ties ? d_en_redo.as<uint32_t>() : nullptr;
  uint32_t* const redo_b = full_ties ? d_en_redo.as<uint32_t>() + 4 + 2 * REDO_CAP : nullptr;
  double* const qrow_all = full_ties ? d_en_qrow.as<double>() : nullptr;
  auto launch_redo = [&](uint32_t* redo, int which, hipStream_t q) {
    if (!redo) return;
    const size_t b0 = n_big_blocks + (size_t)which * REDO_GRID;
    launch_k4_enum_redo(REDO_GRID, q, P, redo, REDO_CAP, d_en_scr.as<int8_t>() + (size_t)stride * b0, stride, qrow_all + (size_t)qstride * b0, qstride,
                        d_jb, d_obj, d_sb, d_en_st.as<unsigned long long>(),
                        which == 0 ? 0u : (uint32_t)std::max(0, dbg.redo_lds));
  };
  long long* const d_rbest = d_en_rbest.as<long long>();
  unsigned long long* const d_st = d_en_st.as<unsigned long long>();
  const uint32_t post_lds = c.post_lds; const PostIn& pin = c.pin; const PostLut& plut = c.plut;
  auto launch = [&](const size_t* cnt, const uint32_t* win) -> hipError_t {
    const bool fork = cnt[CL_STREAM] && (cnt[CL_BITS] || cnt[CL_BIG]);
    hipStream_t const qb = fork ? aux : stream;
    hipError_t e = hipSuccess;
    if (fork) { if ((e = hipEventRecord(ev_fork, stream)) != hipSuccess) return e; if ((e = hipStreamWaitEvent(aux, ev_fork, 0)) != hipSuccess) return e; }
    if (cnt[CL_STREAM]) {
      launch_k4_enum_reg((unsigned)cnt[CL_STREAM], lds_need[CL_STREAM], stream, P, d_sp + s_off[CL_STREAM], (int32_t)n_w[CL_STREAM], per_of[CL_STREAM], d_jb, d_obj, d_sb, d_st, d_rbest, redo_a, REDO_CAP);
      if (!win) {
        launch_redo(redo_a, 0, stream);
        launch_k4_enum_resolve((unsigned)n_w[CL_STREAM], res_lds[CL_STREAM], stream, P, d_sp + s_off[CL_STREAM], d_jb, d_obj, d_sb, d_st);
      }
    }
    if (cnt[CL_BITS]) launch_k4_enum_bits((unsigned)cnt[CL_BITS], lds_need[CL_BITS], qb, P, d_sp + s_off[CL_BITS], (int32_t)n_w[CL_BITS], per_of[CL_BITS], d_jb, d_obj, d_sb, d_st, d_rbest, redo_b, REDO_CAP);
    if (!win && c.async_mode) {
      if (cnt[CL_STREAM]) { if ((e = hipEventRecord(ev_gate[0], stream)) != hipSuccess) return e; gate_set[0] = true; }
      if (fork && cnt[CL_BITS]) { if ((e = hipEventRecord(ev_gate[1], qb)) != hipSuccess) return e; gate_set[1] = true; }
      else if (!fork && cnt[CL_BITS]) { if ((e = hipEventRecord(ev_gate[0], stream)) != hipSuccess) return e; gate_set[0] = true; }
    }
    if (!win) {
      if (nps_a && (e = launch_k4_post(2 * LCR_BLOCK, (unsigned)nps_a, post_lds, stream, pin, d_psl, (int32_t)nps_a, plut)) != hipSuccess) return e;
      if (cnt[CL_BITS]) { launch_redo(redo_b, 1, qb); launch_k4_enum_resolve((unsigned)n_w[CL_BITS], res_lds[CL_BITS], qb, P, d_sp + s_off[CL_BITS], d_jb, d_obj, d_sb, d_st); }
      if (nps_b && (e = launch_k4_post(2 * LCR_BLOCK, (unsigned)nps_b, post_lds, qb, pin, d_psl + nps_a, (int32_t)nps_b, plut)) != hipSuccess) return e;
    }
    if (cnt[CL_BIG]) launch_k4_enum_big((unsigned)cnt[CL_BIG], qb, P, d_sp + s_off[CL_BIG], (int32_t)n_w[CL_BIG], per_of[CL_BIG], d_jb, d_obj, win, d_sb, d_st, qrow_all, qstride);
    if (fork) { if ((e = hipEventRecord(ev_join, aux)) != hipSuccess) return e; if ((e = hipStreamWaitEvent(stream, ev_join, 0)) != hipSuccess) return e; }
    return e;
  };
  PCHK(launch(n_t, nullptr));
  HT("en:launched");
  if (n_w[CL_BIG]) {
    const size_t only_big[NCLS] = {0, 0, n_w[CL_BIG]};
    const int64_t tstride = (big_emax + 63) & ~(int64_t)63;
    PCHK(d_en_terms.reserve((size_t)std::max<int64_t>(tstride, 64) * n_w[CL_BIG] * 8 + 64));
    launch_k4_enum_resolve_big((int32_t)n_w[CL_BIG], stream, P, d_sp + s_off[CL_BIG], d_jb, d_obj, d_sb, d_st, d_win, d_en_terms.as<double>(), tstride);
    PCHK(launch(only_big, d_win));
  }
// ... 268 lines not shown
```

longcallr_amd/csrc/k4_types.h:

```cpp
#pragma once
#include "lcr_dev.h"

struct RegionDev {
  int32_t R, S;
  int32_t rp_off;
  int32_t cp_off;
  int64_t e_off;
  int32_t sig_off;
  int32_t snp_off;
  uint64_t seed;
  long long f_total;
  int32_t F_all;
  int32_t pad_;
};

struct PhaseDev {
  const RegionDev* reg;
  const int32_t* prow_ptr; const int32_t* pcol; const uint8_t* pval;
  const int32_t* ccol_ptr; const int32_t* crow; const uint8_t* cval;
  const uint8_t* snp_fp; const int8_t* snp_vt; const uint8_t* snp_cons;
  const long long* snp_const;
  int8_t* st_sigma; int8_t* st_delta; int8_t* st_eta; long long* st_obj;
  int8_t* scratch; int32_t scratch_stride;
  int32_t lds_state;
  int32_t lds_mat;
  PhaseLutDev lut;
  const struct PostLut* lut64;
  unsigned long long* tie_ctr;
  int32_t tie_arith;
  int32_t enum_elide;
  const int32_t* draw_ord;
};
__device__ __forceinline__ uint64_t draw_row(const int32_t* ord, int row) { return ord ? (uint64_t)ord[row] : (uint64_t)row; }
enum { TIE_SIGMA_F64 = 0,
       TIE_SIGMA_FLIPS = 1,
       TIE_DELTA_UNRES = 2,
       TIE_STEP_UNRES = 3,
       TIE_BEST_F64 = 4,
       TIE_BEST_UNRES = 5,
       TIE_SIGMA_UNRES = 6,
       TIE_STEP_F64 = 7,
       TIE_NCTR = 8 };
#ifdef ENUM_PROF
#define TIE_COUNT(ctr, which, n) do { } while (0)
#else
#define TIE_COUNT(ctr, which, n) atomicAdd(&(ctr)[which], (n))
#endif

struct StageStat { int32_t R, E, max_n, max_rows, E_all, W; };
struct PostLut { double le[31], l1e[31]; double p_homref, p_homvar, log_theta, log2; };


struct ChainDesc {
  int32_t slot;
  int32_t W;
  int64_t tbl_off;
  int64_t adj_off;
  int64_t part_off;
  int32_t n_parts;
  int32_t fast_lds;
  int32_t batch_lds;
  int32_t term_off;
};
struct GridCtl { unsigned arrive, gen, flag[2]; unsigned long long acc[2]; int slot; unsigned pad_[7]; };
struct ChainDev {
  PhaseDev P;
  const ChainDesc* desc;
  const int64_t* row_ptr; const int32_t* col; const uint8_t* val;
  const lcr_candidate* cand; const int32_t* cand_off; const int32_t* row_region_off;
  const int32_t* prow_src;
  uint32_t* ld_tbl; int32_t* ld_adj; int32_t* part_cnt;
  int32_t* adj_ptr; int32_t* blk_ptr; int32_t* blk_of; int32_t* blk_pos; int32_t* blk_nodes;
  int32_t* stack; int32_t* queue; uint8_t* seen; uint8_t* ld_ok; int8_t* new_hap;
  double* qs; double* qfs;
  int32_t* blk_info;
  int32_t* flipcol; int32_t* erow; int32_t* cent;
  int8_t* w_sigma; int8_t* w_delta; int8_t* w_eta; unsigned long long* macc;
  unsigned long long* sig_words;
  GridCtl* ctl;
  unsigned long long* spec_sig; int8_t* spec_de; long long* spec_res; GridCtl* spec_ctl;
  int32_t spec_lanes, spec_ng, spec_s8;
  uint32_t* pk_csr; uint32_t* pk_csc; int64_t pk_cap;
  uint32_t* bt_pk4; int32_t* bt_up4; uint32_t* bt_bs32; int32_t* bt_perm; int32_t* bt_inv; uint8_t* bt_sig8; uint32_t* bt_m32; void* bt_ctl; int64_t bt_cap4; int32_t spec_batch;
  int32_t* tie_flag; double* tie_qrow; double* tie_qsnp; int8_t* tie_ch;
  double* tie_terms;
  long long* dbg;
  double le[31], l1e[31], p_homref, p_homvar, log_theta, log2;
};


struct StageIn {
  const int64_t* row_ptr; const int32_t* col; const uint8_t* val; const uint32_t* links;
  const lcr_candidate* cand; const int32_t* cand_off; const int32_t* row_region_off; const int64_t* start0;
  uint32_t min_linkers, max_enum_snps; uint64_t seed;
  int64_t grid_min;
  const uint8_t* sampled;
};
struct StageOut {
  RegionDev* reg; StageStat* stat;
  int32_t* prow_ptr; int32_t* pcol; uint8_t* pval; int32_t* ccol_ptr; int32_t* crow; uint8_t* cval;
  uint8_t* snp_fp; int8_t* snp_vt; uint8_t* snp_cons; long long* snp_const; int32_t* cursor;
  int32_t* prow_src;
  int32_t* prow_ord;
};
struct PostScratch {
  double *sps, *rpa, *rpb; uint32_t *sflags, *soflags; int32_t *parent, *ccptr;
  int32_t *rptr, *ecol, *erow, *cent; uint8_t* ev;
  int8_t* tag; uint8_t *asg, *fp, *lok, *dirty; int8_t *shap, *sgt, *svt; uint8_t* rcode;
  int32_t* pcnt; int32_t n_parts, pad_;
  int32_t *fdirt, *minf, *ndraw, *gwords;
  GridCtl* ctl;
};
struct PostIn {
  const int64_t* row_ptr; const int32_t* col; const uint8_t* val; const uint32_t* links;
  lcr_candidate* cand; const int32_t* cand_off; const int32_t* row_region_off; const int64_t* start0;
  const int8_t* st_sigma; const int8_t* st_delta; const int8_t* st_eta;
  int8_t* haplotag; uint8_t* assignment; uint32_t* phase_set;
  uint32_t* d_rec;
  const long long* st_obj; long long* h_obj; lcr_candidate* h_cand;
  uint32_t min_linkers, max_enum_snps; uint64_t seed; double cutoff; float min_phase_score;
  long long* dbg_clk;
  const RegionDev* reg; const int32_t* prow_src;
  const uint8_t* sampled;
};
```

longcallr_amd/csrc/lcr_api.hip:

```cpp
#include <chrono>
#include <cmath>
#include <cstdlib>
#include <map>
#include <mutex>

#include "lcr_ctx.h"

namespace {
struct BlockCache {
  std::mutex mu;
  std::multimap<size_t, void*> blocks[2][16];
  size_t held[2][16] = {};
  size_t limit[2] = {(size_t)24 << 30, (size_t)2 << 30};
};
BlockCache& block_cache() { static BlockCache* c = new BlockCache(); return *c; }
}
void* lcr_cache_take(int host, size_t want, size_t* cap) {
  int dev = 0;
  if (hipGetDevice(&dev) != hipSuccess || dev < 0 || dev >= 16) return nullptr;
  BlockCache& bc = block_cache();
  std::lock_guard<std::mutex> g(bc.mu);
  auto& m = bc.blocks[host ? 1 : 0][dev];
  auto it = m.lower_bound(want);
  if (it == m.end() || it->first > 2 * want + (1u << 20)) return nullptr;
// ... 281 lines not shown
}

int lcr_discover_regions(lcr_ctx* c, int32_t mem, int32_t n_reads, const int32_t* ref_start, const int32_t* ref_end,
                         int64_t contig_len, lcr_region_list* out) {
  return lcr_discover_regions_truncated(c, mem, n_reads, ref_start, ref_end, contig_len, 0, 0, out, nullptr);
}

int lcr_discover_regions_truncated(lcr_ctx* c, int32_t mem, int32_t n_reads, const int32_t* ref_start, const int32_t* ref_end,
                                   int64_t contig_len, int32_t truncation, uint32_t truncation_coverage, lcr_region_list* out, int64_t* n_truncated) {
  if (!c || !out || n_reads < 0 || contig_len < 0 || contig_len > 0x7FFFFFF0ll) return LCR_E_ARG;
  if (n_truncated) *n_truncated = 0;
  const uint32_t cap = truncation ? truncation_coverage : UINT32_MAX;
  HIPCHK(c, hipSetDevice(c->device));
  c->rl_start0.clear(); c->rl_len.clear(); c->rl_max.clear();
  out->n_regions = 0; out->start0 = nullptr; out->len = nullptr; out->max_cov = nullptr;
  if (n_reads == 0 || contig_len == 0) return LCR_OK;
  const int32_t *d_s = ref_start, *d_e = ref_end;
  if (mem == LCR_MEM_HOST) {
    HIPCHK(c, c->rd_start.reserve((size_t)n_reads * 4)); HIPCHK(c, c->rd_end.reserve((size_t)n_reads * 4));
    { int rc2 = upload_bytes(c, c->rd_start.p, ref_start, (size_t)n_reads * 4); if (rc2) return rc2; rc2 = upload_bytes(c, c->rd_end.p, ref_end, (size_t)n_reads * 4); if (rc2) return rc2; }
    d_s = c->rd_start.as<int32_t>(); d_e = c->rd_end.as<int32_t>();
  }
  int64_t w_lo = contig_len, w_hi = 0;
  if (mem == LCR_MEM_HOST) {
    for (int32_t r = 0; r < n_reads; r++) {
      const int64_t s = ref_start[r], e = std::min<int64_t>(ref_end[r], contig_len);
      if (s >= 0 && s < e) { w_lo = std::min(w_lo, s); w_hi = std::max(w_hi, e); }
    }
  } else {
    HIPCHK(c, c->rd_cnt.reserve(16));
    int32_t init[2] = {INT_MAX, 0}, got[2] = {INT_MAX, 0};
    HIPCHK(c, hipMemcpyAsync(c->rd_cnt.p, init, 8, hipMemcpyHostToDevice, c->stream));
    launch_k5_span_window(d_s, d_e, n_reads, contig_len, c->rd_cnt.as<int32_t>(), c->stream);
    HIPCHK(c, hipMemcpyAsync(got, c->rd_cnt.p, 8, hipMemcpyDeviceToHost, c->stream));
    HIPCHK(c, hipStreamSynchronize(c->stream));
    if (got[1] > 0) { w_lo = got[0]; w_hi = got[1]; }
  }
  if (w_hi <= w_lo) return LCR_OK;
  const int64_t full_len = contig_len;
  contig_len = w_hi - w_lo;
  const size_t nd = (size_t)contig_len + 2;
  HIPCHK(c, c->rd_diff.reserve(nd * 4)); HIPCHK(c, c->rd_ex.reserve((nd + 1) * 4));
  HIPCHK(c, hipMemsetAsync(c->rd_diff.p, 0, nd * 4, c->stream));
  launch_k5_span_diff(d_s, d_e, n_reads, full_len, w_lo, c->rd_diff.as<uint32_t>(), c->stream);
  launch_scan_i32(c->scan_tmp, (const int32_t*)c->rd_diff.p, c->rd_ex.as<int32_t>(), (int32_t)nd, nullptr, c->stream);
  const int32_t nb = (int32_t)((contig_len + 1023) / 1024);
  HIPCHK(c, c->rd_cnt.reserve(((size_t)nb + 1) * 4)); HIPCHK(c, c->rd_off.reserve(((size_t)nb + 2) * 4));
  uint32_t* d_trunc = truncation ? c->rd_off.as<uint32_t>() + nb + 1 : nullptr;
  if (d_trunc) HIPCHK(c, hipMemsetAsync(d_trunc, 0, 4, c->stream));
  launch_k5_bounds(false, c->rd_ex.as<int32_t>(), contig_len, cap, nb, c->rd_cnt.as<int32_t>(), nullptr, nullptr, nullptr, nullptr, 0, d_trunc, c->stream);
  launch_scan_i32(c->scan_tmp, c->rd_cnt.as<int32_t>(), c->rd_off.as<int32_t>(), nb, c->rd_off.as<int32_t>() + nb, c->stream);
  int32_t tot[2] = {0, 0};
  HIPCHK(c, hipMemcpyAsync(tot, c->rd_off.as<int32_t>() + nb, d_trunc ? 8 : 4, hipMemcpyDeviceToHost, c->stream));
  HIPCHK(c, hipStreamSynchronize(c->stream));
  HIPCHK(c, hipGetLastError());
  const int32_t n_isl = tot[0];
  if (n_truncated) *n_truncated = (int64_t)(uint32_t)tot[1];
  if (n_isl == 0) return LCR_OK;
  const int32_t n_keys = 2 * n_isl + 1;
  HIPCHK(c, c->rd_s.reserve((size_t)n_isl * 4)); HIPCHK(c, c->rd_e.reserve((size_t)n_isl * 4)); HIPCHK(c, c->rd_max.reserve((size_t)n_keys * 4));
  HIPCHK(c, hipMemsetAsync(c->rd_max.p, 0, (size_t)n_keys * 4, c->stream));
  launch_k5_bounds(true, c->rd_ex.as<int32_t>(), contig_len, cap, nb, nullptr, c->rd_off.as<int32_t>(), c->rd_s.as<int32_t>(), c->rd_e.as<int32_t>(),
                   c->rd_max.as<uint32_t>(), n_keys, nullptr, c->stream);
  std::vector<int32_t> hs(n_isl), he(n_isl);
  std::vector<uint32_t> hm(n_keys);
  HIPCHK(c, hipMemcpyAsync(hs.data(), c->rd_s.p, (size_t)n_isl * 4, hipMemcpyDeviceToHost, c->stream));
  HIPCHK(c, hipMemcpyAsync(he.data(), c->rd_e.p, (size_t)n_isl * 4, hipMemcpyDeviceToHost, c->stream));
  HIPCHK(c, hipMemcpyAsync(hm.data(), c->rd_max.p, (size_t)n_keys * 4, hipMemcpyDeviceToHost, c->stream));
  HIPCHK(c, hipStreamSynchronize(c->stream));
  HIPCHK(c, hipGetLastError());
  uint32_t running = 0;
  int64_t pend = -1;
  for (int i = 0; i < n_isl; i++) {
    hs[i] += (int32_t)w_lo; he[i] += (int32_t)w_lo;
    running = std::max(running, std::max(hm[2 * i], hm[2 * i + 1]));
    if (pend < 0) pend = hs[i];
    if ((int64_t)he[i] > pend) {
      c->rl_start0.push_back(pend); c->rl_len.push_back((int32_t)(he[i] - pend + 1)); c->rl_max.push_back(running);
      pend = -1; running = 0;
    }
  }
  out->n_regions = (int32_t)c->rl_start0.size();
  out->start0 = c->rl_start0.data(); out->len = c->rl_len.data(); out->max_cov = c->rl_max.data();
  return LCR_OK;
}

int lcr_get_phase_result(lcr_ctx* c, lcr_phase_result* out) {
  if (!c || !out) return LCR_E_ARG;
  if (c->stage < ST_PHASED) { c->err = "lcr_get_phase_result before lcr_phase"; return LCR_E_STATE; }
  { int rc = phase_settle(c); if (rc) return rc; }
  out->n_rows = c->n_rows; out->n_regions = c->bv.n_regions;
  out->haplotag = c->phase.r_haplotag; out->assignment = c->phase.r_assignment;
  out->phase_set = c->phase.r_phase_set; out->objective = c->phase.objective.data();
  return LCR_OK;
}

int lcr_get_read_records_device(lcr_ctx* c, const lcr_read_record** dev_rec, int32_t* n_rows) {
  if (!c || !dev_rec || !n_rows) return LCR_E_ARG;
  if (c->stage < ST_PHASED) { c->err = "lcr_get_read_records_device before lcr_phase"; return LCR_E_STATE; }
  HIPCHK(c, hipSetDevice(c->device));
  { int rc = phase_settle(c); if (rc) return rc; }
  static_assert(sizeof(lcr_read_record) == 12, "lcr_read_record is 12 bytes");
  *dev_rec = c->phase.d_read_rec.as<lcr_read_record>();
  *n_rows = c->n_rows;
  return LCR_OK;
}

int lcr_collect_phase(lcr_ctx* c, lcr_phase_collected* out) {
  if (!c || !out) return LCR_E_ARG;
  if (!c->res_valid) { c->err = "lcr_collect_phase: no phase results (call it after lcr_phase and before the next lcr_candidates)"; return LCR_E_STATE; }
  HIPCHK(c, hipSetDevice(c->device));
  { int rc = phase_settle(c); if (rc) return rc; }
  out->n_regions = c->res_ng; out->n_rows = c->n_rows; out->n_cand = (int32_t)c->h_cand.size(); out->pad_ = 0;
  out->cand = c->h_cand.data(); out->cand_region_off = c->h_cand_off.data(); out->row_region_off = c->h_row_region_off.data();
  out->haplotag = c->phase.r_haplotag; out->assignment = c->phase.r_assignment; out->phase_set = c->phase.r_phase_set;
  out->objective = c->phase.objective.data();
  out->dev_cand = c->d_cand.as<lcr_candidate>(); out->dev_read_rec = c->phase.d_read_rec.as<lcr_read_record>();
  return LCR_OK;
}

int lcr_ctx_set_async_phase(lcr_ctx* c, int on) {
  if (!c) return LCR_E_ARG;
  HIPCHK(c, hipSetDevice(c->device));
  { int rc = phase_settle(c); if (rc) return rc; }
  c->phase.dbg.async_phase = on != 0;
  if (on) {
    const char* q = getenv("GPU_MAX_HW_QUEUES");
    if (!q || atoi(q) < 8) {
      c->err = "asynchronous phase stage: GPU_MAX_HW_QUEUES is unset or below 8 in this process's environment -- the HIP runtime then shares hardware queues "
               "between the stage's streams (results are the same, the overlap is lost); export GPU_MAX_HW_QUEUES=8 before the process starts";
      return LCR_W_HW_QUEUES;
    }
  }
  return LCR_OK;
}

int lcr_ctx_set_lock_dir(lcr_ctx* c, const char* dir) {
  if (!c || !dir) return LCR_E_ARG;
  c->phase.lock_dir = dir;
  return LCR_OK;
}

int lcr_debug_set(lcr_ctx* c, const char* key, int64_t value) {
  if (!c || !key) return LCR_E_ARG;
  PhaseDebug& d = c->phase.dbg;
  const std::string k(key);
  if (k == "phase_prof") d.prof = (int)value;
  else if (k == "grid_min_entries") d.grid_min = value;
  else if (k == "grid_generic") d.grid_generic = (int)value;
  else if (k == "post_half") d.post_half = (int)value;
  else if (k == "enum_force_big") d.enum_force_big = (int)value;
  else if (k == "enum_force_stream") d.enum_force_stream = (int)value;
  else if (k == "enum_elide") d.enum_elide = value != 0;
  else if (k == "async_phase") d.async_phase = value != 0;
  else if (k == "host_trace") g_lcr_host_trace = value != 0;
  else if (k == "own_fill") g_lcr_own_fill = value != 0;
  else if (k == "fill_selftest") {
    HIPCHK(c, hipSetDevice(c->device));
    const size_t N = 4096;
    DevBuf buf;
    struct Drain { hipStream_t s; ~Drain() { (void)hipStreamSynchronize(s); } } drain{c->stream};
    HIPCHK(c, buf.reserve(4 * N));
    std::vector<uint8_t> host(4 * N), want(4 * N);
    for (size_t off = 0; off < 18; off++)
      for (size_t len : {(size_t)0, (size_t)1, (size_t)15, (size_t)16, (size_t)17, (size_t)255, (size_t)1000 + off, (size_t)2049}) {
        HIPCHK(c, hipMemsetAsync(buf.p, 0xAB, 4 * N, c->stream));
        std::fill(want.begin(), want.end(), (uint8_t)0xAB);
        uint8_t* base = buf.as<uint8_t>();
        HIPCHK(c, lcr_fill_async(base + off, 0x5C, len, c->stream));
        std::fill(want.begin() + off, want.begin() + off + len, (uint8_t)0x5C);
        void* const ptrs[4] = {base + N + off, base + 2 * N + 3, nullptr, base + 3 * N + off};
        const int vals[4] = {0x80, 0, 7, 0xFF};
        const size_t sizes[4] = {len, 33, 0, len / 2};
        HIPCHK(c, lcr_fill_multi_async(4, ptrs, vals, sizes, c->stream));
        std::fill(want.begin() + N + off, want.begin() + N + off + len, (uint8_t)0x80);
        std::fill(want.begin() + 2 * N + 3, want.begin() + 2 * N + 3 + 33, (uint8_t)0);
        std::fill(want.begin() + 3 * N + off, want.begin() + 3 * N + off + len / 2, (uint8_t)0xFF);
        HIPCHK(c, hipMemcpyAsync(host.data(), buf.p, 4 * N, hipMemcpyDeviceToHost, c->stream));
        HIPCHK(c, hipStreamSynchronize(c->stream));
        if (host != want) { c->err = "fill_selftest: a fill kernel wrote other bytes than asked (offset " + std::to_string(off) + ", length " + std::to_string(len) + ")"; return LCR_E_DEVICE; }
      }
  }
  else if (k == "chain_ties") d.chain_ties = value != 0;
  else if (k == "redo_lds") d.redo_lds = (int)std::max<int64_t>(0, std::min<int64_t>(value, 128 * 1024));
  else if (k == "tie_arith") d.tie_arith = (int)std::max<int64_t>(0, std::min<int64_t>(value, 3));
  else if (k == "timing_mask") c->timing_mask = (uint32_t)value;
  else if (k == "hist_tiles") c->dbg_hist_tiles = value > 0 ? 1 : value < 0 ? -1 : 0;
  else if (k == "k3_hits") c->dbg_k3_hits = value != 0;
  else if (k == "fuse_filter") c->dbg_fuse_filter = value != 0;
  else if (k == "spec_compact") c->dbg_spec_compact = value != 0;
  else if (k == "lean_planes") c->dbg_lean_planes = value != 0;
  else if (k == "poison_planes") c->dbg_poison_planes = value != 0;
  else if (k == "grid_spec_batch") d.spec_batch = (int)value;
  else if (k == "grid_spec_lanes") d.spec_lanes = (int)std::max<int64_t>(1, std::min<int64_t>(value, 16));
  else { c->err = "lcr_debug_set: unknown key " + k; return LCR_E_ARG; }
  return LCR_OK;
}

int lcr_get_ld_blocks(lcr_ctx* c, int32_t region, int32_t* n_blocks, const int32_t** block_off, const int32_t** snp_idx) {
  if (!c || !n_blocks || !block_off || !snp_idx) return LCR_E_ARG;
  if (c->stage < ST_PHASED) { c->err = "lcr_get_ld_blocks before lcr_phase"; return LCR_E_STATE; }
  if (region < 0 || region >= c->bv.n_regions) { c->err = "lcr_get_ld_blocks: no such region"; return LCR_E_ARG; }
  { int rc = phase_settle(c); if (rc) return rc; }
  PhaseInputs in;
  in.n_regions = c->bv.n_regions;
  in.cand_region_off = c->h_cand_off.data();
  const int rc = c->phase.ld_blocks(in, region, &c->ld_off, &c->ld_snps, c->stream, &c->err);
  if (rc != LCR_OK) return rc;
  *n_blocks = (int32_t)c->ld_off.size() - 1; *block_off = c->ld_off.data(); *snp_idx = c->ld_snps.data();
  return LCR_OK;
}

int lcr_get_tie_census(lcr_ctx* c, uint64_t out[8]) {
  if (!c || !out) return LCR_E_ARG;
  if (c->stage < ST_PHASED) { c->err = "lcr_get_tie_census before lcr_phase"; return LCR_E_STATE; }
  { int rc = phase_settle(c); if (rc) return rc; }
  for (int i = 0; i < 8; i++) out[i] = i < TIE_NCTR ? (uint64_t)c->phase.tie_census[i] : 0;
  return LCR_OK;
}

}
```

longcallr_amd/csrc/lcr_phase_host.h:

```cpp
#pragma once
#include <string>

#include "lcr_dev.h"
#include "k4_types.h"

struct PhaseInputs {
  int32_t n_regions = 0, n_rows = 0;
  int64_t nnz = 0;
  const int32_t* row_region_off = nullptr;
  const int32_t* cand_region_off = nullptr;
  const int64_t* region_start0 = nullptr;
  const int64_t* region_e_off = nullptr;
  const int64_t* d_row_ptr = nullptr;
  const int32_t* d_col = nullptr;
  const uint8_t* d_val = nullptr;
  const uint32_t* d_row_links = nullptr;
  std::vector<lcr_candidate>* cand = nullptr;
  const lcr_candidate* d_cand = nullptr;
  const int32_t* d_cand_off = nullptr;
  const int32_t* d_row_region_off = nullptr;
  const int64_t* d_start0 = nullptr;
  uint32_t ds_depth = 0; uint64_t ds_seed = 0; const uint8_t* ds_rows = nullptr;
  int snps(int g) const { return cand_region_off[g + 1] - cand_region_off[g]; }
};

struct PhaseDebug {
  int prof = 0;
  long long grid_min = -1;
  int grid_generic = 0;
  int post_half = 0;
  int enum_force_big = 0;
  int enum_force_stream = 0;
  int enum_elide = 1;
  int spec_batch = 1;
  int spec_lanes = 8;
  int redo_lds = 64 * 1024;
  int chain_ties = 1;
  int tie_arith = 3;
  int async_phase = 0;
};

struct PhaseCall;

struct PhaseHost {
  PhaseDebug dbg;
  std::string lock_dir;
  std::vector<double> objective;
  const int8_t* r_haplotag = nullptr;
  const uint8_t* r_assignment = nullptr;
  const uint32_t* r_phase_set = nullptr;
  DevBuf d_reg, d_prow_ptr, d_pcol, d_pval, d_ccol_ptr, d_crow, d_cval, d_snp, d_snp_const, d_cur, d_prow_src;
  DevBuf d_sampled, d_prow_ord; HostBuf h_sampled, h_smp_slots;
  std::vector<uint8_t> ds_applied;
  bool ds_any = false;
  int32_t ds_ng = 0, ds_nrow = 0;
  DevBuf d_grid_ctl, d_grid_tot;
  DevBuf d_st_enum, d_st_chain, d_read_rec, d_lut64, d_tie, d_prof_clk;
  bool lut64_ready = false;
  DevBuf d_ch_desc, d_ch_slots, d_ch_tbl, d_ch_adj, d_ch_part, d_ch_snpi, d_ch_snpb, d_ch_q, d_ch_info, d_ch_rowi, d_ch_enti, d_ch_work, d_ch_macc, d_ch_sig;
  DevBuf d_spec_sig, d_spec_de, d_spec_res, d_pk, d_bt;
  DevBuf d_tie_flag, d_tie_q, d_tie_ch, d_tie_terms;
  DevBuf d_en_job, d_en_obj, d_en_st, d_en_rbest, d_en_scr, d_en_qrow, d_en_redo, d_en_terms;
  DevBuf d_gp_snp, d_gp_ent, d_gp_part;
  HostBuf h_stat, h_res, h_cand_obj, h_census, h_en_up, h_ch_up;
  unsigned long long tie_census[TIE_NCTR] = {0, 0, 0, 0, 0, 0, 0, 0};
  hipStream_t side = nullptr;
  hipEvent_t ev_in = nullptr, ev_csr = nullptr, ev_fork = nullptr, ev_join = nullptr;
  hipStream_t aux = nullptr;
  hipStream_t main_q = nullptr, q_first = nullptr;
  hipEvent_t ev_gate[2] = {nullptr, nullptr};
  bool gate_set[2] = {false, false};
  hipError_t gate_stream(hipStream_t s) {
    if (!pending) return hipSuccess;
    for (int k = 0; k < 2; k++) if (gate_set[k]) { hipError_t e = hipStreamWaitEvent(s, ev_gate[k], 0); if (e != hipSuccess) return e; }
    return hipSuccess;
  }
  hipEvent_t ev_user = nullptr;
  bool pending = false;
  struct Pending {
    int ng = 0;
    std::vector<int32_t> cand_off;
    size_t res_ps = 0, res_tag = 0, res_asg = 0, hc_obj = 0;
    std::vector<lcr_candidate>* cand = nullptr;
  } pend;
  int settle(std::string* err);
  ChainDev chain_dev{};
  std::vector<ChainDesc> chain_desc;
  std::vector<uint64_t> enum_keys;
  std::vector<int64_t> enum_job_base, enum_st_base;
  int ld_blocks(const PhaseInputs& in, int region, std::vector<int32_t>* off, std::vector<int32_t>* snps, hipStream_t s, std::string* err);
  int run(const PhaseInputs& in, const lcr_params& p, hipStream_t s, std::string* err);
  int open_queues(PhaseCall& c), size_buffers(PhaseCall& c), sample(PhaseCall& c), stage(PhaseCall& c), classify(PhaseCall& c), wait_sizes(PhaseCall& c);
  int launch_enum(PhaseCall& c), launch_chain(PhaseCall& c), launch_gpost(PhaseCall& c), report_prof(PhaseCall& c);
  bool mark_pending(PhaseCall& c);
  void release() {
    for (hipStream_t* q : {&side, &aux, &main_q}) { if (*q) (void)hipStreamDestroy(*q); *q = nullptr; }
    for (hipEvent_t* e : {&ev_in, &ev_csr, &ev_fork, &ev_join, &ev_user, &ev_gate[0], &ev_gate[1]}) { if (*e) (void)hipEventDestroy(*e); *e = nullptr; }
    gate_set[0] = gate_set[1] = false;
    pending = false;
  }
};
```

Before: 6.662 billion.

## Precompute per-region enum LDS image once and bulk-copy it in enum_bits blocks

Adds a k4_enum_image kernel that builds each region's LDS staging image (LUTs, CSC/CSR packing, permutation, per-SNP constants) once into global memory, tagged by R/E/S and a serial. Each k4_enum_bits tile block for that region then copies the image into LDS with wide 16-byte loads instead of redoing the ballot-heavy staging. This removes repeated setup work across the many tiles of one region, at the cost of an extra kernel launch, global memory for the images, and a tag check. It is enabled by default, with a debug knob to turn it off and another to poison the buffer.

```diff
diff --git a/longcallr_amd/api.py b/longcallr_amd/api.py
--- a/longcallr_amd/api.py
+++ b/longcallr_amd/api.py
@@ -22,7 +22,7 @@
 
 _DEBUG_ENV = {"LCR_PHASE_PROF": "phase_prof", "LCR_GRID_MIN_ENTRIES": "grid_min_entries",
               "LCR_GRID_GENERIC": "grid_generic", "LCR_GRID_SPEC_LANES": "grid_spec_lanes", "LCR_GRID_SPEC_BATCH": "grid_spec_batch", "LCR_POST_HALF": "post_half", "LCR_ENUM_FORCE_BIG": "enum_force_big",
-              "LCR_ENUM_FORCE_STREAM": "enum_force_stream", "LCR_ENUM_ELIDE": "enum_elide", "LCR_HIST_TILES": "hist_tiles", "LCR_TIE_ARITH": "tie_arith", "LCR_CHAIN_TIES": "chain_ties", "LCR_K3_HITS": "k3_hits", "LCR_FUSE_FILTER": "fuse_filter", "LCR_ASYNC_PHASE": "async_phase", "LCR_HOST_TRACE": "host_trace", "LCR_OWN_FILL": "own_fill", "LCR_REDO_LDS": "redo_lds", "LCR_SPEC_COMPACT": "spec_compact", "LCR_LEAN_PLANES": "lean_planes"}
+              "LCR_ENUM_FORCE_STREAM": "enum_force_stream", "LCR_ENUM_ELIDE": "enum_elide", "LCR_ENUM_IMAGE": "enum_image", "LCR_HIST_TILES": "hist_tiles", "LCR_TIE_ARITH": "tie_arith", "LCR_CHAIN_TIES": "chain_ties", "LCR_K3_HITS": "k3_hits", "LCR_FUSE_FILTER": "fuse_filter", "LCR_ASYNC_PHASE": "async_phase", "LCR_HOST_TRACE": "host_trace", "LCR_OWN_FILL": "own_fill", "LCR_REDO_LDS": "redo_lds", "LCR_SPEC_COMPACT": "spec_compact", "LCR_LEAN_PLANES": "lean_planes"}
 
 
 class Engine:
diff --git a/longcallr_amd/csrc/k4_enum.hip b/longcallr_amd/csrc/k4_enum.hip
--- a/longcallr_amd/csrc/k4_enum.hip
+++ b/longcallr_amd/csrc/k4_enum.hip
@@ -43,7 +43,16 @@
 #define ENUM_STEP(k) do { } while (0)
 #define ENUM_STEP_FLUSH(base) do { } while (0)
 #endif
-#if defined(ENUM_PROF) && !defined(ENUM_PROF_STEPS)
+#if defined(ENUM_PROF) && ENUM_PROF == 3
+#define ENUM_PROF_STAGE 1
+#define ENUM_STAGE_T(v) const long long v = (long long)wall_clock64()
+#define ENUM_STAGE_FLUSH(t0, t1) do { if (threadIdx.x == 0) { const long long t2_ = (long long)wall_clock64(); atomicAdd(&P.tie_ctr[0], (unsigned long long)((t1) - (t0))); \
+  atomicAdd(&P.tie_ctr[1], (unsigned long long)(t2_ - (t0))); atomicAdd(&P.tie_ctr[2], 1ull); } } while (0)
+#else
+#define ENUM_STAGE_T(v) do { } while (0)
+#define ENUM_STAGE_FLUSH(t0, t1) do { } while (0)
+#endif
+#if defined(ENUM_PROF) && !defined(ENUM_PROF_STEPS) && !defined(ENUM_PROF_STAGE)
 #define ENUM_PROF_TIMES 1
 #define ENUM_PT(i) do { if (threadIdx.x == 0) atomicMax(&P.tie_ctr[i], (unsigned long long)((long long)wall_clock64() - prof_t0)); } while (0)
 #else
@@ -798,6 +807,122 @@
 __device__ __forceinline__ uint32_t enum_spread8(uint32_t x) { x = (x | (x << 4)) & 0x0F0Fu; x = (x | (x << 2)) & 0x3333u; x = (x | (x << 1)) & 0x5555u; return x; }
 __device__ __forceinline__ int enum_mad24(int a, int b, int c) { int d; asm("v_mad_i32_i24 %0, %1, %2, %3" : "=v"(d) : "v"(a), "v"(b), "v"(c)); return d; }
 
+__device__ __forceinline__ void enum_stage_bits(const PhaseDev& P, const RegionDev& rd, const EnumLayout& L, const uint32_t E, uint8_t* const lds, EnumImageHdr& H) {
+  const int R = rd.R, S = rd.S;
+  uint2* wl2 = (uint2*)lds;
+  double* lut = (double*)(lds + L.lut);
+  uint2* csr = (uint2*)(lds + L.csr);
+  uint32_t* csc = (uint32_t*)(lds + L.csc);
+  uint16_t* rp = (uint16_t*)(lds + L.rp);
+  uint16_t* ent16 = (uint16_t*)(lds + L.ent16);
+  const int tid = threadIdx.x, nt = blockDim.x;
+  if (tid < 32) {
+    const long long w = tid < 31 ? P.lut.f1e[tid] - P.lut.fe[tid] : 0;
+    wl2[tid] = make_uint2((uint32_t)w & 0x7fffffu, (uint32_t)(w >> 23) & 0xffffffu);
+  }
+  if (tid < 64) lut[tid] = (tid & 31) < 31 ? (tid < 32 ? P.lut64->le[tid] : P.lut64->l1e[tid - 32]) : 0.0;
+  const int32_t* g_rp = P.prow_ptr + rd.rp_off;
+  for (int r = tid; r <= R; r += nt) rp[r] = (uint16_t)g_rp[r];
+  if (tid <= S && tid < 33) H.cps[tid] = P.ccol_ptr[rd.cp_off + tid];
+  int eta_init = 0;
+  if (tid < 32) {
+    long long cF = 0, cW = 0, cRef = 0, cVar = 0, het = 0; bool live = false;
+    if (tid < S) {
+      const long long* sc = P.snp_const + 4ll * (rd.snp_off + tid);
+      cF = sc[0]; cW = sc[1]; cRef = sc[2] + P.lut.f_homref; cVar = sc[3] + P.lut.f_homvar;
+      const int n = P.ccol_ptr[rd.cp_off + tid + 1] - P.ccol_ptr[rd.cp_off + tid];
+      het = P.lut.f_het0 - (long long)n * P.lut.f_log2;
+      live = P.snp_fp[rd.snp_off + tid] != 0 && n > 0;
+      eta_init = init_genotype(P.snp_vt[rd.snp_off + tid]);
+    }
+    H.cF[tid] = cF; H.cW[tid] = cW; H.cRef[tid] = cRef; H.cVar[tid] = cVar; H.het[tid] = het; H.live[tid] = live ? 1 : 0;
+  }
+  if (tid < 64) {
+    const uint32_t a = (uint32_t)__ballot(tid < S && tid < 32 && eta_init == 0), b = (uint32_t)__ballot(tid < S && tid < 32 && eta_init == 1);
+    if (tid == 0) { H.e0i = a; H.epi = b; }
+  }
+  __syncthreads();
+  for (int e = tid; e < (int)E; e += nt) {
+    const uint32_t cv = P.cval[rd.e_off + e];
+    int col = 0;
+    for (int i = 0; i < S; i++) col += (int)((uint32_t)e >= (uint32_t)H.cps[i + 1]);
+    csc[e] = (uint32_t)P.crow[rd.e_off + e] | ((uint32_t)col << 16) | ((cv & 32u) << 16) | ((cv & 31u) << 22) | 0x80000000u;
+  }
+  uint16_t* const perm = (uint16_t*)(lds + L.pos);
+  uint16_t* const gof = perm + ((R + 3) & ~3);
+  uint16_t* const kidx = (uint16_t*)(lds + L.state);
+  __syncthreads();
+  if (tid < 64) {
+    const int ln = tid;
+    const unsigned long long lt = (1ull << ln) - 1ull;
+    int nS = 0;
+    int tot[32];
+#pragma unroll
+    for (int Lk = 0; Lk < 32; Lk++) tot[Lk] = 0;
+    for (int base = 0; base < R; base += 64) {
+      const int r = base + ln;
+      const int n = r < R ? min(31, (int)rp[r + 1] - (int)rp[r]) : 0;
+      const unsigned long long bs = __ballot(n == 1);
+      if (n == 1) kidx[r] = (uint16_t)(nS + __popcll(bs & lt));
+      nS += __popcll(bs);
+      if (__ballot(n >= 2)) {
+#pragma unroll
+        for (int Lk = 2; Lk < 32; Lk++) {
+          if (Lk <= S) {
+            const unsigned long long bm = __ballot(n == Lk);
+            if (n == Lk) kidx[r] = (uint16_t)(tot[Lk] + __popcll(bm & lt));
+            tot[Lk] += __popcll(bm);
+          }
+        }
+      }
+    }
+    int mine = 0;
+#pragma unroll
+    for (int Lk = 2; Lk < 32; Lk++) if (ln == Lk) mine = tot[Lk];
+    int longer = 0;
+    for (int Lk = 31; Lk >= 2; Lk--) { const int tl = __shfl(mine, Lk, 64); if (ln == Lk) H.lstart[ln] = longer; longer += tl; }
+    if (ln == 0) { H.cnt[0] = longer; H.cnt[2] = nS; }
+  }
+  __syncthreads();
+  const int nM = H.cnt[0], nS = H.cnt[2], nG = (nM + 63) >> 6;
+  for (int r = tid; r < R; r += nt) {
+    const int n = min(31, (int)rp[r + 1] - (int)rp[r]);
+    if (n >= 2) perm[H.lstart[n] + kidx[r]] = (uint16_t)r;
+  }
+  __syncthreads();
+  if (tid < 64) {
+    int carry = 0;
+    for (int g0 = 0; g0 <= nG; g0 += 64) {
+      const int g = g0 + tid;
+      const int len = g < nG ? min(31, (int)rp[perm[64 * g] + 1] - (int)rp[perm[64 * g]]) : 0;
+      const int inc = wave_incl_scan(len);
+      if (g <= nG) gof[g] = (uint16_t)(carry + inc - len);
+      carry += __builtin_amdgcn_readlane(inc, 63);
+    }
+  }
+  __syncthreads();
+  const int eM = 64 * (int)gof[nG];
+  for (int x = tid; x < eM; x += nt) csr[x] = make_uint2(0u, 0u);
+  __syncthreads();
+  for (int r = tid; r < R; r += nt) {
+    const int e0 = rp[r], e1 = rp[r + 1];
+    if (e0 == e1) continue;
+    int at, step;
+    if (e1 - e0 >= 2) {
+      const int k = H.lstart[min(31, e1 - e0)] + kidx[r];
+      at = 64 * (int)gof[k >> 6] + (k & 63); step = 64;
+    } else { perm[nM + kidx[r]] = (uint16_t)r; at = eM + kidx[r]; step = 1; }
+    for (int e = e0; e < e1; e++) {
+      const uint32_t v = P.pval[rd.e_off + e];
+      const uint32_t meta = (uint32_t)P.pcol[rd.e_off + e] | (v & 32u) | (e + 1 == e1 ? 64u : 0u) | 128u;
+      const uint2 w = wl2[v & 31u];
+      csr[at + (e - e0) * step] = make_uint2(w.x | (meta << 24), w.y);
+      ent16[e] = (uint16_t)((meta & 63u) | ((v & 31u) << 6) | (e + 1 == e1 ? 0x800u : 0u));
+    }
+  }
+  __syncthreads();
+}
+
 #ifndef ENUM_BITS_OCC
 #define ENUM_BITS_OCC 2
 #endif
@@ -809,6 +934,7 @@
              long long* __restrict__ job_obj, const int64_t* __restrict__ st_base, unsigned long long* __restrict__ st_words,
              long long* __restrict__ region_best, uint32_t* __restrict__ redo, uint32_t redo_cap) {
   extern __shared__ __attribute__((aligned(16))) uint8_t lds[];
+  ENUM_STAGE_T(prof_ts0);
   const EnumTile t = enum_tile_of(P, spans, n_spans, per, false);
   const RegionDev rd = P.reg[t.slot];
   const int R = rd.R, S = rd.S;
@@ -823,117 +949,33 @@
   uint16_t* ent16 = (uint16_t*)(lds + L.ent16);
   const int tid = threadIdx.x, nt = blockDim.x;
   const uint32_t c = enum_chunk(E);
-  __shared__ long long s_cF[32], s_cW[32], s_cRef[32], s_cVar[32], s_het[32];
-  __shared__ uint8_t s_live[32];
-  if (tid < 32) {
-    const long long w = tid < 31 ? P.lut.f1e[tid] - P.lut.fe[tid] : 0;
-    wl2[tid] = make_uint2((uint32_t)w & 0x7fffffu, (uint32_t)(w >> 23) & 0xffffffu);
-  }
-  if (tid < 64) lut[tid] = (tid & 31) < 31 ? (tid < 32 ? P.lut64->le[tid] : P.lut64->l1e[tid - 32]) : 0.0;
-  const int32_t* g_rp = P.prow_ptr + rd.rp_off;
-  for (int r = tid; r <= R; r += nt) rp[r] = (uint16_t)g_rp[r];
-  __shared__ int32_t cps[33];
-  if (tid <= S && tid < 33) cps[tid] = P.ccol_ptr[rd.cp_off + tid];
-  int eta_init = 0;
-  if (tid < 32) {
-    long long cF = 0, cW = 0, cRef = 0, cVar = 0, het = 0; bool live = false;
-    if (tid < S) {
-      const long long* sc = P.snp_const + 4ll * (rd.snp_off + tid);
-      cF = sc[0]; cW = sc[1]; cRef = sc[2] + P.lut.f_homref; cVar = sc[3] + P.lut.f_homvar;
-      const int n = P.ccol_ptr[rd.cp_off + tid + 1] - P.ccol_ptr[rd.cp_off + tid];
-      het = P.lut.f_het0 - (long long)n * P.lut.f_log2;
-      live = P.snp_fp[rd.snp_off + tid] != 0 && n > 0;
-      eta_init = init_genotype(P.snp_vt[rd.snp_off + tid]);
-    }
-    s_cF[tid] = cF; s_cW[tid] = cW; s_cRef[tid] = cRef; s_cVar[tid] = cVar; s_het[tid] = het; s_live[tid] = live ? 1 : 0;
-  }
-  __shared__ uint32_t s_e0i, s_epi;
-  if (tid < 64) {
-    const uint32_t a = (uint32_t)__ballot(tid < S && tid < 32 && eta_init == 0), b = (uint32_t)__ballot(tid < S && tid < 32 && eta_init == 1);
-    if (tid == 0) { s_e0i = a; s_epi = b; }
-  }
-  __syncthreads();
-  for (int e = tid; e < (int)E; e += nt) {
-    const uint32_t cv = P.cval[rd.e_off + e];
-    int col = 0;
-    for (int i = 0; i < S; i++) col += (int)((uint32_t)e >= (uint32_t)cps[i + 1]);
-    csc[e] = (uint32_t)P.crow[rd.e_off + e] | ((uint32_t)col << 16) | ((cv & 32u) << 16) | ((cv & 31u) << 22) | 0x80000000u;
-  }
-  uint16_t* const perm = (uint16_t*)(lds + L.pos);
-  uint16_t* const gof = perm + ((R + 3) & ~3);
-  uint16_t* const kidx = (uint16_t*)(lds + L.state);
-  __shared__ int s_cnt[3];
-  __shared__ int s_lstart[32];
-  __syncthreads();
-  if (tid < 64) {
-    const int ln = tid;
-    const unsigned long long lt = (1ull << ln) - 1ull;
-    int nS = 0;
-    int tot[32];
-#pragma unroll
-    for (int Lk = 0; Lk < 32; Lk++) tot[Lk] = 0;
-    for (int base = 0; base < R; base += 64) {
-      const int r = base + ln;
-      const int n = r < R ? min(31, (int)rp[r + 1] - (int)rp[r]) : 0;
-      const unsigned long long bs = __ballot(n == 1);
-      if (n == 1) kidx[r] = (uint16_t)(nS + __popcll(bs & lt));
-      nS += __popcll(bs);
-      if (__ballot(n >= 2)) {
-#pragma unroll
-        for (int Lk = 2; Lk < 32; Lk++) {
-          if (Lk <= S) {
-            const unsigned long long bm = __ballot(n == Lk);
-            if (n == Lk) kidx[r] = (uint16_t)(tot[Lk] + __popcll(bm & lt));
-            tot[Lk] += __popcll(bm);
-          }
-        }
-      }
-    }
-    int mine = 0;
-#pragma unroll
-    for (int Lk = 2; Lk < 32; Lk++) if (ln == Lk) mine = tot[Lk];
-    int longer = 0;
-    for (int Lk = 31; Lk >= 2; Lk--) { const int tl = __shfl(mine, Lk, 64); if (ln == Lk) s_lstart[ln] = longer; longer += tl; }
-    if (ln == 0) { s_cnt[0] = longer; s_cnt[2] = nS; }
-  }
-  __syncthreads();
-  const int nM = s_cnt[0], nS = s_cnt[2], nG = (nM + 63) >> 6;
-  for (int r = tid; r < R; r += nt) {
-    const int n = min(31, (int)rp[r + 1] - (int)rp[r]);
-    if (n >= 2) perm[s_lstart[n] + kidx[r]] = (uint16_t)r;
-  }
-  __syncthreads();
-  if (tid < 64) {
-    int carry = 0;
-    for (int g0 = 0; g0 <= nG; g0 += 64) {
-      const int g = g0 + tid;
-      const int len = g < nG ? min(31, (int)rp[perm[64 * g] + 1] - (int)rp[perm[64 * g]]) : 0;
-      const int inc = wave_incl_scan(len);
-      if (g <= nG) gof[g] = (uint16_t)(carry + inc - len);
-      carry += __builtin_amdgcn_readlane(inc, 63);
-    }
-  }
-  __syncthreads();
+  __shared__ __attribute__((aligned(16))) EnumImageHdr s_hdr;
+  bool have_image = false;
+  if (P.enum_image) {
+    const uint4 tg = P.enum_tag[t.slot];
+    have_image = tg.x == (uint32_t)R && tg.y == E && tg.z == (uint32_t)S && tg.w == P.enum_serial;
+  }
+  if (have_image) {
+    constexpr uint32_t HQ = sizeof(EnumImageHdr) / 16;
+    const uint4* const src = (const uint4*)(P.enum_image + (uint64_t)t.slot * P.enum_image_stride);
+    uint4* const hdst = (uint4*)&s_hdr; uint4* const ldst = (uint4*)lds;
+    const uint32_t nq = HQ + L.state / 16;
+    for (uint32_t q0 = (uint32_t)tid; q0 < nq; q0 += 8u * (uint32_t)nt) {
+      uint4 v[8];
+#pragma unroll
+      for (uint32_t u = 0; u < 8; u++) v[u] = src[min(q0 + u * (uint32_t)nt, nq - 1u)];
+#pragma unroll
+      for (uint32_t u = 0; u < 8; u++) { const uint32_t q = q0 + u * (uint32_t)nt; if (q < nq) { if (q < HQ) hdst[q] = v[u]; else ldst[q - HQ] = v[u]; } }
+    }
+    __syncthreads();
+  } else enum_stage_bits(P, rd, L, E, lds, s_hdr);
+  ENUM_STAGE_T(prof_ts1);
+  const long long* const s_cF = s_hdr.cF; const long long* const s_cW = s_hdr.cW; const long long* const s_cRef = s_hdr.cRef;
+  const long long* const s_cVar = s_hdr.cVar; const long long* const s_het = s_hdr.het; const uint8_t* const s_live = s_hdr.live;
+  const uint16_t* const perm = (const uint16_t*)(lds + L.pos);
+  const uint16_t* const gof = perm + ((R + 3) & ~3);
+  const int nM = s_hdr.cnt[0], nS = s_hdr.cnt[2], nG = (nM + 63) >> 6;
   const int eM = 64 * (int)gof[nG];
-  for (int x = tid; x < eM; x += nt) csr[x] = make_uint2(0u, 0u);
-  __syncthreads();
-  for (int r = tid; r < R; r += nt) {
-    const int e0 = rp[r], e1 = rp[r + 1];
-    if (e0 == e1) continue;
-    int at, step;
-    if (e1 - e0 >= 2) {
-      const int k = s_lstart[min(31, e1 - e0)] + kidx[r];
-      at = 64 * (int)gof[k >> 6] + (k & 63); step = 64;
-    } else { perm[nM + kidx[r]] = (uint16_t)r; at = eM + kidx[r]; step = 1; }
-    for (int e = e0; e < e1; e++) {
-      const uint32_t v = P.pval[rd.e_off + e];
-      const uint32_t meta = (uint32_t)P.pcol[rd.e_off + e] | (v & 32u) | (e + 1 == e1 ? 64u : 0u) | 128u;
-      const uint2 w = wl2[v & 31u];
-      csr[at + (e - e0) * step] = make_uint2(w.x | (meta << 24), w.y);
-      ent16[e] = (uint16_t)((meta & 63u) | ((v & 31u) << 6) | (e + 1 == e1 ? 0x800u : 0u));
-    }
-  }
-  __syncthreads();
   const int lane = tid & 63, wave = tid >> 6;
   uint8_t* const wst = lds + L.state + wave * L.stride;
   uint8_t* const sg8 = wst;
@@ -947,7 +989,7 @@
   const int c0 = min((int)E, lane * (int)c), c1 = min((int)E, (lane + 1) * (int)c);
   const int n_del = (int)min(c, E);
   const uint32_t smask = S >= 32 ? 0xffffffffu : ((1u << S) - 1u);
-  const uint32_t e0_init = s_e0i, ep_init = s_epi;
+  const uint32_t e0_init = s_hdr.e0i, ep_init = s_hdr.epi;
   const int nk = (R + 63) / 64;
   unsigned long long* const st_reg = st_words + st_base[t.slot];
   const uint32_t stw = enum_state_words((uint32_t)R);
@@ -1322,6 +1364,34 @@
     if (n_step) TIE_COUNT(P.tie_ctr, TIE_STEP_UNRES, (unsigned long long)n_step);
   }
   ENUM_STEP_FLUSH(0);
+  ENUM_STAGE_FLUSH(prof_ts0, prof_ts1);
+}
+
+__global__ void __launch_bounds__(64 * ENUM_WAVES)
+k4_enum_image(PhaseDev P, uint32_t max_enum_snps, uint32_t lds_cap, uint8_t* __restrict__ image, uint4* __restrict__ tag) {
+  extern __shared__ __attribute__((aligned(16))) uint8_t lds[];
+  __shared__ __attribute__((aligned(16))) EnumImageHdr s_hdr;
+  const int slot = blockIdx.x;
+  const RegionDev rd = P.reg[slot];
+  const int R = rd.R, S = rd.S;
+  const int tid = threadIdx.x, nt = blockDim.x;
+  bool ok = S >= 1 && (uint32_t)S <= min(max_enum_snps, 31u) && R >= 0 && R < 65536;
+  uint32_t E = 0;
+  if (ok) { E = (uint32_t)P.prow_ptr[rd.rp_off + R]; ok = E < 65536u; }
+  EnumLayout L{};
+  if (ok) {
+    L = enum_layout((uint32_t)R, E, true, (uint32_t)S);
+    ok = L.total <= ENUM_LDS_MAX && L.total <= lds_cap && (uint64_t)sizeof(EnumImageHdr) + L.state <= P.enum_image_stride;
+  }
+  if (!ok) { if (tid == 0) tag[slot] = make_uint4(0u, 0u, 0u, 0u); return; }
+  enum_stage_bits(P, rd, L, E, lds, s_hdr);
+  constexpr uint32_t HQ = sizeof(EnumImageHdr) / 16;
+  uint4* const dst = (uint4*)(image + (uint64_t)slot * P.enum_image_stride);
+  const uint4* const hsrc = (const uint4*)&s_hdr; const uint4* const lsrc = (const uint4*)lds;
+  const uint32_t nq = HQ + L.state / 16;
+  for (uint32_t q = (uint32_t)tid; q < nq; q += (uint32_t)nt) dst[q] = q < HQ ? hsrc[q] : lsrc[q - HQ];
+  __syncthreads();
+  if (tid == 0) tag[slot] = make_uint4((uint32_t)R, E, (uint32_t)S, P.enum_serial);
 }
 
 __device__ __forceinline__ void enum_big_restart(const PhaseDev& P, const RegionDev& rd, int slot, uint32_t e, bool winner, int8_t* base, double* qrow,
@@ -1531,6 +1601,9 @@
                          long long* region_best, uint32_t* redo, uint32_t redo_cap) {
   hipLaunchKernelGGL(k4_enum_bits, dim3(n_blocks), dim3(64 * ENUM_WAVES), dyn_lds, s, P, spans, n_spans, per, job_base, job_obj, st_base, st_words, region_best, redo, redo_cap);
 }
+void launch_k4_enum_image(int32_t n_regions, uint32_t dyn_lds, hipStream_t s, const PhaseDev& P, uint32_t max_enum_snps, uint8_t* image, uint4* tag) {
+  hipLaunchKernelGGL(k4_enum_image, dim3((unsigned)n_regions), dim3(64 * ENUM_WAVES), dyn_lds, s, P, max_enum_snps, dyn_lds, image, tag);
+}
 void launch_k4_enum_redo(unsigned n_blocks, hipStream_t s, const PhaseDev& P, const uint32_t* redo, uint32_t redo_cap, int8_t* scratch, int32_t scratch_stride,
                          double* qrow, int64_t qrow_stride, const int64_t* job_base, long long* job_obj, const int64_t* st_base, unsigned long long* st_words,
                          uint32_t lds_bytes) {
diff --git a/longcallr_amd/csrc/k4_kernels.h b/longcallr_amd/csrc/k4_kernels.h
--- a/longcallr_amd/csrc/k4_kernels.h
+++ b/longcallr_amd/csrc/k4_kernels.h
@@ -11,11 +11,11 @@
 #define ENUM_BITS_PER_V 64
 #endif
 constexpr uint32_t ENUM_BITS_PER = ENUM_BITS_PER_V;
-__host__ __device__ inline uint32_t enum_bits_sp(uint32_t S) { return (S + 7) & ~7u; }
-__host__ __device__ inline uint32_t enum_bits_stride(uint32_t R, uint32_t S) { return ((R + 15) & ~7u) + 8 * 8 * enum_bits_sp(S) + 8 * 32 + 4 * 24 + 4 * (ENUM_TQ + 2); }
+__host__ __device__ constexpr uint32_t enum_bits_sp(uint32_t S) { return (S + 7) & ~7u; }
+__host__ __device__ constexpr uint32_t enum_bits_stride(uint32_t R, uint32_t S) { return ((R + 15) & ~7u) + 8 * 8 * enum_bits_sp(S) + 8 * 32 + 4 * 24 + 4 * (ENUM_TQ + 2); }
 struct EnumLayout { uint32_t lut, csr, csc, rp, first_row, ent16, pos, state, stride, total; };
-__host__ __device__ inline EnumLayout enum_layout(uint32_t R, uint32_t E, bool bits = false, uint32_t S = 32) {
-  EnumLayout L;
+__host__ __device__ constexpr EnumLayout enum_layout(uint32_t R, uint32_t E, bool bits = false, uint32_t S = 32) {
+  EnumLayout L{};
   uint32_t o = 256;
   L.lut = o; o += 512;
   L.csr = o; o += 8 * (E + (bits ? 64 * (S < 31 ? S : 31) : 0));
@@ -32,6 +32,17 @@
   L.total = o;
   return L;
 }
+struct EnumImageHdr {
+  long long cF[32], cW[32], cRef[32], cVar[32], het[32];
+  int32_t cps[36];
+  int32_t lstart[32];
+  int32_t cnt[4];
+  uint32_t e0i, epi, pad_[2];
+  uint8_t live[32];
+};
+static_assert(sizeof(EnumImageHdr) % 16 == 0, "an image is copied 16 bytes at a time");
+static_assert(enum_layout(1, 1, true, 1).state % 16 == 0 && enum_layout(1023, 4097, true, 31).state % 16 == 0 && ENUM_LDS_MAX % 16 == 0, "an image is copied 16 bytes at a time");
+void launch_k4_enum_image(int32_t n_regions, uint32_t dyn_lds, hipStream_t s, const PhaseDev& P, uint32_t max_enum_snps, uint8_t* image, uint4* tag);
 __host__ __device__ inline uint32_t enum_state_words(uint32_t R) { return (R + 63) / 64 + 3; }
 __host__ __device__ inline uint32_t resolve_tlcap(uint32_t S) { return S >= 12 ? 4096u : (S < 6 ? 64u : (1u << S)); }
 struct ResolveLayout { uint32_t lut, rp, ent16, pse, sg_ref, hetw, repmask, rowsnps, res, total; };
diff --git a/longcallr_amd/csrc/k4_phase.hip b/longcallr_amd/csrc/k4_phase.hip
--- a/longcallr_amd/csrc/k4_phase.hip
+++ b/longcallr_amd/csrc/k4_phase.hip
@@ -176,6 +176,7 @@
   std::vector<uint8_t> grid_post;
   uint32_t post_lds = 0;
   size_t gp_S = 1, gp_rows = 1, gp_E = 1;
+  uint64_t img_stride = 0; uint32_t img_lds = 0;
   GridLock grid_lock;
   PhaseCall(const PhaseInputs& in_, const lcr_params& prm_, hipStream_t user_stream, std::string* err_, bool prof_)
       : in(in_), prm(prm_), err(err_), sq(user_stream), ng(in_.n_regions), nrow(in_.n_rows), ncand(in_.cand_region_off[in_.n_regions]),
@@ -364,6 +365,21 @@
       c.gp_S = std::max(c.gp_S, (size_t)S); c.gp_rows = std::max(c.gp_rows, (size_t)nr_g); c.gp_E = std::max(c.gp_E, (size_t)E_all);
     } else c.post_lds = std::max(c.post_lds, need);
   }
+  if (dbg.enum_image) {
+    for (int g : c.enum_slots) {
+      const int S = in.snps(g);
+      if (S > 31) continue;
+      const int64_t nr_g = in.row_region_off[g + 1] - in.row_region_off[g], E_all = in.region_e_off[g + 1] - in.region_e_off[g];
+      uint32_t total = ENUM_LDS_MAX, state = ENUM_LDS_MAX;
+      if (nr_g < 65536 && E_all < 65536) {
+        const EnumLayout EL = enum_layout((uint32_t)nr_g, (uint32_t)E_all, true, (uint32_t)S);
+        if (EL.total <= ENUM_LDS_MAX) { total = EL.total; state = EL.state; }
+      }
+      c.img_lds = std::max(c.img_lds, total);
+      c.img_stride = std::max<uint64_t>(c.img_stride, sizeof(EnumImageHdr) + (uint64_t)state);
+    }
+    if (c.img_stride) PCHK(d_en_img.reserve((((size_t)c.ng * 16 + 255) & ~(size_t)255) +(size_t)c.ng * c.img_stride));
+  }
   return LCR_OK;
 }
 
@@ -382,6 +398,14 @@
     PCHK(hipEventRecord(ev_csr, sq));
   }
   if (c.async_mode) { PCHK(hipEventRecord(ev_user, sq)); PCHK(hipStreamWaitEvent(c.stream, ev_user, 0)); }
+  if (dbg.poison_enum_image && d_en_img.p) PCHK(lcr_fill_async(d_en_img.p, 0xA5, d_en_img.cap, c.stream));
+  if (c.img_stride) {
+    const size_t tag_bytes = ((size_t)c.ng * 16 + 255) & ~(size_t)255;
+    c.P.enum_tag = d_en_img.as<uint4>(); c.P.enum_image = d_en_img.as<uint8_t>() + tag_bytes;
+    c.P.enum_image_stride = c.img_stride; c.P.enum_serial = ++enum_serial;
+    launch_k4_enum_image((int32_t)c.ng, c.img_lds, c.stream, c.P, c.prm.max_enum_snps, d_en_img.as<uint8_t>() + tag_bytes, d_en_img.as<uint4>());
+    PCHK(hipGetLastError());
+  }
   HT("ph:presync");
   if (c.ng) PCHK(hipStreamSynchronize(sq));
   HT("ph:synced");
diff --git a/longcallr_amd/csrc/k4_types.h b/longcallr_amd/csrc/k4_types.h
--- a/longcallr_amd/csrc/k4_types.h
+++ b/longcallr_amd/csrc/k4_types.h
@@ -30,6 +30,9 @@
   int32_t tie_arith;
   int32_t enum_elide;
   const int32_t* draw_ord;
+  const uint8_t* enum_image; const uint4* enum_tag;
+  uint64_t enum_image_stride;
+  uint32_t enum_serial, pad_;
 };
 __device__ __forceinline__ uint64_t draw_row(const int32_t* ord, int row) { return ord ? (uint64_t)ord[row] : (uint64_t)row; }
 enum { TIE_SIGMA_F64 = 0,
diff --git a/longcallr_amd/csrc/lcr_api.hip b/longcallr_amd/csrc/lcr_api.hip
--- a/longcallr_amd/csrc/lcr_api.hip
+++ b/longcallr_amd/csrc/lcr_api.hip
@@ -457,6 +457,8 @@
   else if (k == "enum_force_big") d.enum_force_big = (int)value;
   else if (k == "enum_force_stream") d.enum_force_stream = (int)value;
   else if (k == "enum_elide") d.enum_elide = value != 0;
+  else if (k == "enum_image") d.enum_image = value != 0;
+  else if (k == "poison_enum_image") d.poison_enum_image = value != 0;
   else if (k == "async_phase") d.async_phase = value != 0;
   else if (k == "host_trace") g_lcr_host_trace = value != 0;
   else if (k == "own_fill") g_lcr_own_fill = value != 0;
diff --git a/longcallr_amd/csrc/lcr_phase_host.h b/longcallr_amd/csrc/lcr_phase_host.h
--- a/longcallr_amd/csrc/lcr_phase_host.h
+++ b/longcallr_amd/csrc/lcr_phase_host.h
@@ -32,6 +32,8 @@
   int enum_force_big = 0;
   int enum_force_stream = 0;
   int enum_elide = 1;
+  int enum_image = 1;
+  int poison_enum_image = 0;
   int spec_batch = 1;
   int spec_lanes = 8;
   int redo_lds = 64 * 1024;
@@ -61,6 +63,8 @@
   DevBuf d_spec_sig, d_spec_de, d_spec_res, d_pk, d_bt;
   DevBuf d_tie_flag, d_tie_q, d_tie_ch, d_tie_terms;
   DevBuf d_en_job, d_en_obj, d_en_st, d_en_rbest, d_en_scr, d_en_qrow, d_en_redo, d_en_terms;
+  DevBuf d_en_img;
+  uint32_t enum_serial = 0;
   DevBuf d_gp_snp, d_gp_ent, d_gp_part;
   HostBuf h_stat, h_res, h_cand_obj, h_census, h_en_up, h_ch_up;
   unsigned long long tie_census[TIE_NCTR] = {0, 0, 0, 0, 0, 0, 0, 0};
```

Result: no change. 6.730 billion (median of 6 runs) (+1.0%).
